# lawfuyang/HobbyRenderer

Hardware: AMD Instinct MI355X
Metric: Mrays/s at 1920×1080, 8 spp, 4 bounces; 1/2/4/8 GPU scaling (higher is better)
Workload: dtype f32; 1 GPU; config 2: Cornell-box-class procedural scene (38 triangles, 9 instances, closed room, emissive quad + default sun), 1920x1080, 8 spp (accumulation indices 0..7), 4 bounces; frames_in_flight=2, serial_kernels=False, mode=default

## Files before the change

### hobbyrenderer_amd/csrc/pt_device.h

```cpp
#pragma once

#include <hip/hip_runtime.h>
#include <stdint.h>

#include "../../include/hobbyrt_pt.h"
#include "../../include/hobbyrt/detmath.h"
#include "../../include/hobbyrt/srgb_table.h"

#define HRT_DEV __device__ __forceinline__

#if defined(HRPT_PHASE_PROFILE) && defined(HRPT_PHASE_TU)
extern __device__ unsigned long long g_phaseCounters[128];
#define HRT_PHASE(k)                                                                                                      \
    do {                                                                                                                  \
        const unsigned long long m_ = __ballot(true);                                                                     \
        if ((threadIdx.x & 63u) == (unsigned)(__ffsll((long long)m_) - 1)) {                                              \
            atomicAdd(&g_phaseCounters[2 * (k)], 1ull); atomicAdd(&g_phaseCounters[2 * (k) + 1], (unsigned long long)__popcll(m_)); \
        }                                                                                                                 \
    } while (0)
#else
#define HRT_PHASE(k) do { } while (0)
#endif
enum {
    PH_EXT_ITER = 0, PH_EXT_REFILL, PH_EXT_NODE, PH_EXT_LEAF, PH_EXT_TRI, PH_EXT_FINISH, PH_EXT_CANDIDATE,
    PH_ANY_ITER = 8, PH_ANY_REFILL, PH_ANY_NODE, PH_ANY_LEAF, PH_ANY_TRI, PH_ANY_FINISH,
    PH_SHADE_ITER = 16, PH_SHADE_HIT, PH_SHADE_ATTR, PH_SHADE_TEX, PH_SHADE_TRANS, PH_SHADE_NEE, PH_SHADE_LOBE_BEGIN, PH_SHADE_DIFFUSE, PH_SHADE_SPEC,
    PH_SHADE_SKY, PH_SHADE_WRITE, PH_SHADE_SORT,
    PH_SHADOW_ENTRY = 32, PH_SHADOW_SAMPLE, PH_SHADOW_QUERY, PH_SHADOW_CONTRIB, PH_SHADOW_RAYS_ITEM,
    PH_COUNT = 40
};

namespace hrt {

struct f2 { float x, y; };
struct f3 { float x, y, z; };
struct f4 { float x, y, z, w; };

HRT_DEV f3 mk3(float x, float y, float z) { f3 r; r.x = x; r.y = y; r.z = z; return r; }
HRT_DEV f3 mk3(const float* p) { return mk3(p[0], p[1], p[2]); }
HRT_DEV f3 operator+(f3 a, f3 b) { return mk3(a.x + b.x, a.y + b.y, a.z + b.z); }
HRT_DEV f3 operator-(f3 a, f3 b) { return mk3(a.x - b.x, a.y - b.y, a.z - b.z); }
HRT_DEV f3 operator*(f3 a, f3 b) { return mk3(a.x * b.x, a.y * b.y, a.z * b.z); }
HRT_DEV f3 operator*(f3 a, float s) { return mk3(a.x * s, a.y * s, a.z * s); }
HRT_DEV f3 operator/(f3 a, float s) { return mk3(a.x / s, a.y / s, a.z / s); }
HRT_DEV f3 operator-(f3 a) { return mk3(-a.x, -a.y, -a.z); }
HRT_DEV float dot(f3 a, f3 b) { return (a.x * b.x + a.y * b.y) + a.z * b.z; }
HRT_DEV f3 cross(f3 a, f3 b) { return mk3(a.y * b.z - a.z * b.y, a.z * b.x - a.x * b.z, a.x * b.y - a.y * b.x); }
HRT_DEV float length(f3 a) { return hrt_sqrt(dot(a, a)); }
HRT_DEV f3 normalize(f3 a) { float inv = 1.0f / hrt_sqrt(dot(a, a)); return a * inv; }
HRT_DEV float lerp(float a, float b, float t) { return a + t * (b - a); }
HRT_DEV float comp(f3 a, int k) { return k == 0 ? a.x : (k == 1 ? a.y : a.z); }
HRT_DEV float maxcomp(f3 a) { return hrt_max(a.x, hrt_max(a.y, a.z)); }
HRT_DEV f3 reflect(f3 i, f3 n) { float s = 2.0f * dot(i, n); return i - n * s; }
HRT_DEV f3 refract(f3 i, f3 n, float eta)
{
    float d = dot(n, i);
    float k = 1.0f - (eta * eta) * (1.0f - d * d);
    if (k < 0.0f) return mk3(0.0f, 0.0f, 0.0f);
    float s = eta * d + hrt_sqrt(k);
    return i * eta - n * s;
}
HRT_DEV f4 lerp4(f4 a, f4 b, float t)
{
    f4 r; float w = 1.0f - t;
    r.x = a.x * w + b.x * t; r.y = a.y * w + b.y * t; r.z = a.z * w + b.z * t; r.w = a.w * w + b.w * t;
    return r;
}

struct GpuNode {
    float lmin[3]; int32_t left;
    float lmax[3]; int32_t right;
    float rmin[3]; uint32_t pad0;
    float rmax[3]; uint32_t pad1;
};
struct GpuNode4 {
    float4 minx, maxx, miny, maxy, minz, maxz; int4 child; uint4 pad;
};
struct GpuNodeQ {
    float ox, oy, oz, sx;
    uint32_t lox, hix, loy, hiy;
    uint32_t loz, hiz; float sy, sz;
    int32_t child[4];
};
static_assert(sizeof(GpuNodeQ) == 64, "four 16-byte rows");
struct GpuTri {
    float p0[3]; uint32_t inst;
    float p1[3]; uint32_t prim;
    float p2[3]; uint32_t flags;
};
struct GpuTriAttr { float4 a, b, c, d, e; };
struct GpuTriTangent { float4 t0, t1, t2; };
struct GpuInstShade { float4 adj0, adj1, adj2; };
struct GpuInstance {
    float world[12];
    float inv[12];
    int32_t blasRoot; uint32_t flags, material; float boxEps;
    uint32_t mesh; float objMaxAbs, invNorm; uint32_t pad;
};
static_assert(sizeof(GpuInstance) == 128, "bvh_build.h HostInstance");
struct GpuTexture {
    const uint8_t* texels; uint32_t w, h, format, mipCount;
    uint32_t mipOffset[HRPT_TEXTURE_MAX_MIPS];
};

struct SceneView {
    const GpuNode* nodes; uint32_t nodeCount;
    const GpuNode4* nodes4; uint32_t node4Count;
    const GpuNodeQ* nodesQ;
    const GpuTri* tris; uint32_t triCount;
    int32_t rootLeaf;
    const GpuTriAttr* attrs;
    const GpuTriTangent* tangents;
    const GpuInstShade* instShade;
    const HrptMaterialConstants* materials;
    const HrptGPULight* lights; uint32_t lightCount;
    const GpuTexture* textures; uint32_t textureCount;
    const uint16_t* lutTransmittance;
    const uint16_t* lutScattering;
    const GpuInstance* instances; uint32_t instanceCount;
};

struct Ray { f3 o, d; float tmin, tmax; };
struct Hit { float t; uint32_t inst, prim; float u, v; uint32_t opaque; uint32_t tri; bool valid; };
struct HitKey { float t; uint32_t inst, prim; bool have; };

struct RayShear { int kx, ky, kz; float Sx, Sy, Sz; };

HRT_DEV RayShear make_shear(f3 d)
{
    RayShear s;
    int kz = 0;
    if (hrt_abs(d.y) > hrt_abs(comp(d, kz))) kz = 1;
    if (hrt_abs(d.z) > hrt_abs(comp(d, kz))) kz = 2;
    int kx = (kz + 1) % 3, ky = (kx + 1) % 3;
    if (comp(d, kz) < 0.0f) { int t = kx; kx = ky; ky = t; }
    s.kx = kx; s.ky = ky; s.kz = kz;
    float dz = comp(d, kz);
    s.Sx = comp(d, kx) / dz; s.Sy = comp(d, ky) / dz; s.Sz = 1.0f / dz;
    return s;
}
HRT_DEV bool key_less(float t, uint32_t inst, uint32_t prim, float t2, uint32_t inst2, uint32_t prim2)
{
    if (t < t2) return true;
    if (t > t2) return false;
    if (inst < inst2) return true;
    if (inst > inst2) return false;
    return prim < prim2;
}
HRT_DEV bool tri_test(f3 p0, f3 p1, f3 p2, const Ray& r, const RayShear& s, float& t, float& u, float& v)
{
    f3 A = p0 - r.o, B = p1 - r.o, C = p2 - r.o;
    float Akz = comp(A, s.kz), Bkz = comp(B, s.kz), Ckz = comp(C, s.kz);
    float Ax = comp(A, s.kx) - s.Sx * Akz, Ay = comp(A, s.ky) - s.Sy * Akz;
    float Bx = comp(B, s.kx) - s.Sx * Bkz, By = comp(B, s.ky) - s.Sy * Bkz;
    float Cx = comp(C, s.kx) - s.Sx * Ckz, Cy = comp(C, s.ky) - s.Sy * Ckz;
    float U = Cx * By - Cy * Bx;
    float V = Ax * Cy - Ay * Cx;
    float W = Bx * Ay - By * Ax;
    if ((U < 0.0f || V < 0.0f || W < 0.0f) && (U > 0.0f || V > 0.0f || W > 0.0f)) return false;
    float det = (U + V) + W;
    if (det == 0.0f) return false;
    float Az = s.Sz * Akz, Bz = s.Sz * Bkz, Cz = s.Sz * Ckz;
    float T = (U * Az + V * Bz) + W * Cz;
    float rcp = 1.0f / det;
    float tt = T * rcp;
    if (!(tt > r.tmin && tt < r.tmax)) return false;
    t = tt; u = V * rcp; v = W * rcp;
    return true;
}

struct GlobalBvh {
    static constexpr int kWidth = 2; static constexpr bool kTwoLevel = false;
    const GpuNode* nodes; const GpuTri* tris;
    HRT_DEV void node(int i, float4& a, float4& b, float4& c, float4& d) const
    {
        const float4* p = reinterpret_cast<const float4*>(nodes + i);
        a = p[0]; b = p[1]; c = p[2]; d = p[3];
    }
    HRT_DEV void tri(uint32_t i, float4& a, float4& b, float4& c) const
    {
        const float4* p = reinterpret_cast<const float4*>(tris + i);
        a = p[0]; b = p[1]; c = p[2];
    }
};

struct GlobalBvh4 {
    static constexpr int kWidth = 4; static constexpr bool kTwoLevel = false; static constexpr bool kLds = false;
    const GpuNode4* nodes; const GpuTri* tris;
    HRT_DEV void tri(uint32_t i, float4& a, float4& b, float4& c) const
    {
        const float4* p = reinterpret_cast<const float4*>(reinterpret_cast<const char*>(tris) + (size_t)(i * 48u));
        a = p[0]; b = p[1]; c = p[2];
    }
    HRT_DEV uint32_t rowoff(int i, uint32_t byteOffset) const { return (uint32_t)i * 128u + byteOffset; }
    HRT_DEV float4 load(uint32_t off) const { return *reinterpret_cast<const float4*>(reinterpret_cast<const char*>(nodes) + (size_t)off); }
};

struct GlobalBvhQ {
    static constexpr int kWidth = 4; static constexpr bool kTwoLevel = false; static constexpr bool kLds = false; static constexpr bool kQuantised = true;
    const GpuNodeQ* nodes; const GpuTri* tris;
    HRT_DEV void tri(uint32_t i, float4& a, float4& b, float4& c) const
    {
        const float4* p = reinterpret_cast<const float4*>(reinterpret_cast<const char*>(tris) + (size_t)(i * 48u));
        a = p[0]; b = p[1]; c = p[2];
    }
    HRT_DEV float4 row(int i, uint32_t r) const { return *reinterpret_cast<const float4*>(reinterpret_cast<const char*>(nodes) + (size_t)((uint32_t)i * 64u + r * 16u)); }
};
template <class BVH, class = void> struct IsQuantised { static constexpr bool value = false; };
template <class BVH> struct IsQuantised<BVH, decltype((void)BVH::kQuantised)> { static constexpr bool value = true; };

HRT_DEV f3 slab_origin_term(f3 o, f3 inv) { return mk3(-(o.x * inv.x), -(o.y * inv.y), -(o.z * inv.z)); }
HRT_DEV bool slab(float4 bmin, float4 bmax, f3 noi, f3 inv, float t0, float t1, float& tnear)
{
    float tx0 = __builtin_fmaf(bmin.x, inv.x, noi.x), tx1 = __builtin_fmaf(bmax.x, inv.x, noi.x);
    float ty0 = __builtin_fmaf(bmin.y, inv.y, noi.y), ty1 = __builtin_fmaf(bmax.y, inv.y, noi.y);
    float tz0 = __builtin_fmaf(bmin.z, inv.z, noi.z), tz1 = __builtin_fmaf(bmax.z, inv.z, noi.z);
    float lo = __builtin_fmaxf(__builtin_fmaxf(__builtin_fminf(tx0, tx1), __builtin_fminf(ty0, ty1)), __builtin_fmaxf(__builtin_fminf(tz0, tz1), t0));
    float hi = __builtin_fminf(__builtin_fminf(__builtin_fmaxf(tx0, tx1), __builtin_fmaxf(ty0, ty1)), __builtin_fminf(__builtin_fmaxf(tz0, tz1), t1));
    tnear = lo;
    return __builtin_fmaf(-__builtin_fabsf(lo), 2e-6f, lo) <= __builtin_fmaf(__builtin_fabsf(hi), 2e-6f, hi);
}

constexpr int32_t kTraversalDone = (int32_t)0x80000000;

HRT_DEV float slab1(float bminx, float bminy, float bminz, float bmaxx, float bmaxy, float bmaxz, f3 noi, f3 inv, float t0, float t1)
{
    float tx0 = __builtin_fmaf(bminx, inv.x, noi.x), tx1 = __builtin_fmaf(bmaxx, inv.x, noi.x);
    float ty0 = __builtin_fmaf(bminy, inv.y, noi.y), ty1 = __builtin_fmaf(bmaxy, inv.y, noi.y);
    float tz0 = __builtin_fmaf(bminz, inv.z, noi.z), tz1 = __builtin_fmaf(bmaxz, inv.z, noi.z);
    float lo = __builtin_fmaxf(__builtin_fmaxf(__builtin_fminf(tx0, tx1), __builtin_fminf(ty0, ty1)), __builtin_fmaxf(__builtin_fminf(tz0, tz1), t0));
    float hi = __builtin_fminf(__builtin_fminf(__builtin_fmaxf(tx0, tx1), __builtin_fmaxf(ty0, ty1)), __builtin_fminf(__builtin_fmaxf(tz0, tz1), t1));
    bool hit = __builtin_fmaf(-__builtin_fabsf(lo), 2e-6f, lo) <= __builtin_fmaf(__builtin_fabsf(hi), 2e-6f, hi);
    return hit ? lo : __builtin_inff();
}
HRT_DEV void cswap(float& ta, int32_t& ra, float& tb, int32_t& rb)
{
    bool sw = tb < ta;
    float t = sw ? tb : ta; tb = sw ? ta : tb; ta = t;
    int32_t r = sw ? rb : ra; rb = sw ? ra : rb; ra = r;
}

template <class BVH, class STACK>
HRT_DEV int32_t inner_step(const BVH& bvh, int32_t cur, f3 noi, f3 noiF, f3 inv, float tmin, float tlim, STACK& stack, int& sp)
{
    if constexpr (BVH::kWidth == 2) {
        float4 a, b, c, d; bvh.node(cur, a, b, c, d);
        int32_t li = __float_as_int(a.w), ri = __float_as_int(b.w);
        float tl, tr;
        bool hl = slab(a, b, noi, inv, tmin, tlim, tl);
        bool hr = slab(c, d, noi, inv, tmin, tlim, tr);
        if (hl && hr) { bool leftFirst = tl <= tr; stack.push(sp++, leftFirst ? ri : li); return leftFirst ? li : ri; }
        if (hl) return li;
        if (hr) return ri;
        return (sp == 0) ? kTraversalDone : stack.pop(--sp);
    } else if constexpr (IsQuantised<BVH>::value) {
        const float4 r0 = bvh.row(cur, 0u), r1 = bvh.row(cur, 1u), r2 = bvh.row(cur, 2u), chf = bvh.row(cur, 3u);
        const float ax = r0.w * inv.x, ay = r2.z * inv.y, az = r2.w * inv.z;
        const float bx = __builtin_fmaf(r0.x, inv.x, noi.x), by = __builtin_fmaf(r0.y, inv.y, noi.y), bz = __builtin_fmaf(r0.z, inv.z, noi.z);
        const bool negx = inv.x < 0.0f, negy = inv.y < 0.0f, negz = inv.z < 0.0f;
        const uint32_t wnx = __float_as_uint(negx ? r1.y : r1.x), wfx = __float_as_uint(negx ? r1.x : r1.y);
        const uint32_t wny = __float_as_uint(negy ? r1.w : r1.z), wfy = __float_as_uint(negy ? r1.z : r1.w);
        const uint32_t wnz = __float_as_uint(negz ? r2.y : r2.x), wfz = __float_as_uint(negz ? r2.x : r2.y);
        auto boxq = [&](uint32_t sh) {
            const float lo = __builtin_fmaxf(__builtin_fmaxf(__builtin_fmaxf(__builtin_fmaf((float)((wnx >> sh) & 255u), ax, bx), __builtin_fmaf((float)((wny >> sh) & 255u), ay, by)),
                                                             __builtin_fmaf((float)((wnz >> sh) & 255u), az, bz)), tmin);
            const float far3 = __builtin_fminf(__builtin_fminf(__builtin_fmaf((float)((wfx >> sh) & 255u), ax, bx), __builtin_fmaf((float)((wfy >> sh) & 255u), ay, by)),
                                               __builtin_fmaf((float)((wfz >> sh) & 255u), az, bz));
            const float hi = __builtin_fminf(far3, tlim) * (1.0f + 4e-6f);
            return lo <= hi ? lo : __builtin_inff();
        };
        float t0 = boxq(0u), t1 = boxq(8u), t2 = boxq(16u), t3 = boxq(24u);
        int32_t r0i = __float_as_int(chf.x), r1i = __float_as_int(chf.y), r2i = __float_as_int(chf.z), r3i = __float_as_int(chf.w);
        cswap(t0, r0i, t1, r1i); cswap(t2, r2i, t3, r3i); cswap(t0, r0i, t2, r2i); cswap(t1, r1i, t3, r3i); cswap(t1, r1i, t2, r2i);
        const float inf = __builtin_inff();
        if (t3 < inf) stack.push(sp++, r3i);
        if (t2 < inf) stack.push(sp++, r2i);
        if (t1 < inf) stack.push(sp++, r1i);
        if (t0 < inf) return r0i;
        return (sp == 0) ? kTraversalDone : stack.pop(--sp);
    } else {
        const uint32_t nx = inv.x < 0.0f ? 16u : 0u, ny = inv.y < 0.0f ? 48u : 32u, nz = inv.z < 0.0f ? 80u : 64u;
        const uint32_t onx = bvh.rowoff(cur, nx), ony = bvh.rowoff(cur, ny), onz = bvh.rowoff(cur, nz);
        const float4 anx = bvh.load(onx), any = bvh.load(ony), anz = bvh.load(onz);
        const float4 afx = bvh.load(onx ^ 16u), afy = bvh.load(ony ^ 16u), afz = bvh.load(onz ^ 16u);
        const float4 chf = bvh.load(bvh.rowoff(cur, 96u));
        auto box = [&](float bnx, float bny, float bnz, float bfx, float bfy, float bfz) {
            const float lo = __builtin_fmaxf(__builtin_fmaxf(__builtin_fmaxf(__builtin_fmaf(bnx, inv.x, noi.x), __builtin_fmaf(bny, inv.y, noi.y)), __builtin_fmaf(bnz, inv.z, noi.z)), tmin);
            const float far3 = __builtin_fminf(__builtin_fminf(__builtin_fmaf(bfx, inv.x, noiF.x), __builtin_fmaf(bfy, inv.y, noiF.y)), __builtin_fmaf(bfz, inv.z, noiF.z));
            const float hi = __builtin_fminf(far3, tlim) * (1.0f + 4e-6f);
            return lo <= hi ? lo : __builtin_inff();
        };
        float t0 = box(anx.x, any.x, anz.x, afx.x, afy.x, afz.x);
        float t1 = box(anx.y, any.y, anz.y, afx.y, afy.y, afz.y);
        float t2 = box(anx.z, any.z, anz.z, afx.z, afy.z, afz.z);
        float t3 = box(anx.w, any.w, anz.w, afx.w, afy.w, afz.w);
        int32_t r0 = __float_as_int(chf.x), r1 = __float_as_int(chf.y), r2 = __float_as_int(chf.z), r3 = __float_as_int(chf.w);
        cswap(t0, r0, t1, r1); cswap(t2, r2, t3, r3); cswap(t0, r0, t2, r2); cswap(t1, r1, t3, r3); cswap(t1, r1, t2, r2);
        const float inf = __builtin_inff();
        if (t3 < inf) stack.push(sp++, r3);
        if (t2 < inf) stack.push(sp++, r2);
        if (t1 < inf) stack.push(sp++, r1);
        if (t0 < inf) return r0;
        return (sp == 0) ? kTraversalDone : stack.pop(--sp);
    }
}

template <class BVH, class STACK>
HRT_DEV int32_t inner_step(const BVH& bvh, int32_t cur, f3 noi, f3 inv, float tmin, float tlim, STACK& stack, int& sp)
{
    return inner_step(bvh, cur, noi, noi, inv, tmin, tlim, stack, sp);
}

HRT_DEV f3 traversal_rcp(f3 d)
{
    auto one = [](float x) { return __builtin_fminf(__builtin_fmaxf(__builtin_amdgcn_rcpf(x), -1e20f), 1e20f); };
    return mk3(one(d.x), one(d.y), one(d.z));
}

template <class BVH, class STACK>
HRT_DEV Hit closest_any(const BVH& bvh, int32_t rootLeaf, uint32_t nodeCount, const Ray& r, HitKey lower, STACK& stack, uint32_t nodeLoopMin = 0)
{
    Hit best; best.valid = false; best.t = r.tmax; best.inst = 0; best.prim = 0; best.u = 0; best.v = 0; best.opaque = 0; best.tri = 0;
    if (!(r.d.x == r.d.x && r.d.y == r.d.y && r.d.z == r.d.z)) return best;
    RayShear sh = make_shear(r.d);
    f3 inv = traversal_rcp(r.d), noi = slab_origin_term(r.o, inv);
    int sp = 0;
    int32_t cur;
    if (nodeCount == 0) { if (rootLeaf == 0) return best; cur = rootLeaf; }
    else cur = 0;
    float tlim = r.tmax;
    for (;;) {
        while (cur >= 0) {
            cur = inner_step(bvh, cur, noi, inv, r.tmin, tlim, stack, sp);
            if ((uint32_t)__popcll(__ballot(cur >= 0)) < nodeLoopMin) break;
        }
        if (cur == kTraversalDone) break;
        if (cur < 0) {
            uint32_t enc = (uint32_t)(~cur);
            uint32_t first = enc >> 2, count = (enc & 3u) + 1u;
            for (uint32_t i = 0; i < count; ++i) {
                float4 a, b, c; bvh.tri(first + i, a, b, c);
                float t, u, v;
                if (tri_test(mk3(a.x, a.y, a.z), mk3(b.x, b.y, b.z), mk3(c.x, c.y, c.z), r, sh, t, u, v)) {
                    uint32_t inst = __float_as_uint(a.w), prim = __float_as_uint(b.w);
                    bool ok = !lower.have || key_less(lower.t, lower.inst, lower.prim, t, inst, prim);
                    const bool take = ok && (!best.valid || key_less(t, inst, prim, best.t, best.inst, best.prim));
                    best.t = take ? t : best.t; best.u = take ? u : best.u; best.v = take ? v : best.v;
                    best.inst = take ? inst : best.inst; best.prim = take ? prim : best.prim; best.tri = take ? first + i : best.tri;
                    best.opaque = take ? (__float_as_uint(c.w) & 1u) : best.opaque;
                    best.valid = best.valid || take;
                    tlim = take ? t : tlim;
                }
            }
            if (sp == 0) break;
            cur = stack.pop(--sp);
        }
    }
    return best;
}

template <class BVH, class STACK>
HRT_DEV bool any_opaque(const BVH& bvh, int32_t rootLeaf, uint32_t nodeCount, const Ray& r, STACK& stack, bool& sawNonOpaque, uint32_t nodeLoopMin = 0)
{
    sawNonOpaque = false;
    if (!(r.d.x == r.d.x && r.d.y == r.d.y && r.d.z == r.d.z)) return false;
    RayShear sh = make_shear(r.d);
    f3 inv = traversal_rcp(r.d), noi = slab_origin_term(r.o, inv);
    int sp = 0; int32_t cur;
    if (nodeCount == 0) { if (rootLeaf == 0) return false; cur = rootLeaf; }
    else cur = 0;
    for (;;) {
        while (cur >= 0) {
            cur = inner_step(bvh, cur, noi, inv, r.tmin, r.tmax, stack, sp);
            if ((uint32_t)__popcll(__ballot(cur >= 0)) < nodeLoopMin) break;
        }
        if (cur == kTraversalDone) break;
        if (cur < 0) {
            uint32_t enc = (uint32_t)(~cur);
            uint32_t first = enc >> 2, count = (enc & 3u) + 1u;
            for (uint32_t i = 0; i < count; ++i) {
                float4 a, b, c; bvh.tri(first + i, a, b, c);
                float t, u, v;
                if (tri_test(mk3(a.x, a.y, a.z), mk3(b.x, b.y, b.z), mk3(c.x, c.y, c.z), r, sh, t, u, v)) {
                    if (__float_as_uint(c.w) & 1u) return true;
                    sawNonOpaque = true;
                }
            }
            if (sp == 0) break;
            cur = stack.pop(--sp);
        }
    }
    return false;
}

constexpr int32_t kExitBlas = 0x7FFFFFFE;
struct GlobalBvhTl : GlobalBvh4 {
    static constexpr bool kTwoLevel = true;
    const GpuInstance* instances;
};
struct TlCull { f3 inv, noi, noiF; int32_t inst; };
HRT_DEV void tl_world(TlCull& c, const Ray& r)
{
    c.inv = traversal_rcp(r.d); c.noi = slab_origin_term(r.o, c.inv); c.noiF = c.noi; c.inst = -1;
}
HRT_DEV void tl_enter(TlCull& c, const GpuInstance& I, int32_t inst, const Ray& r)
{
    const float4* w = reinterpret_cast<const float4*>(I.world);
    const float4 w2 = w[2];
    const float4* q = reinterpret_cast<const float4*>(I.inv);
    const float4 q0 = q[0], q1 = q[1]; const float q22 = I.inv[8];
    const f3 rel = mk3(r.o.x - w2.y, r.o.y - w2.z, r.o.z - w2.w);
    const f3 oo = mk3(__builtin_fmaf(rel.z, q1.z, __builtin_fmaf(rel.y, q0.w, rel.x * q0.x)),
                      __builtin_fmaf(rel.z, q1.w, __builtin_fmaf(rel.y, q1.x, rel.x * q0.y)),
                      __builtin_fmaf(rel.z, q22, __builtin_fmaf(rel.y, q1.y, rel.x * q0.z)));
    const f3 od = mk3(__builtin_fmaf(r.d.z, q1.z, __builtin_fmaf(r.d.y, q0.w, r.d.x * q0.x)),
                      __builtin_fmaf(r.d.z, q1.w, __builtin_fmaf(r.d.y, q1.x, r.d.x * q0.y)),
                      __builtin_fmaf(r.d.z, q22, __builtin_fmaf(r.d.y, q1.y, r.d.x * q0.z)));
    auto max3abs = [](f3 v) { return __builtin_fmaxf(__builtin_fmaxf(__builtin_fabsf(v.x), __builtin_fabsf(v.y)), __builtin_fabsf(v.z)); };
    const float oMax = __builtin_fmaxf(max3abs(r.o), __builtin_fmaxf(__builtin_fmaxf(__builtin_fabsf(w2.y), __builtin_fabsf(w2.z)), __builtin_fabsf(w2.w)));
    const float dRatio = max3abs(r.d) * I.invNorm / __builtin_fmaxf(max3abs(od), 1e-30f);
    const float eps = I.boxEps + 4.0f * 2.4e-7f * (I.invNorm * (oMax + max3abs(rel)) + dRatio * (I.objMaxAbs + max3abs(oo)));
    c.inv = traversal_rcp(od);
    const f3 n = slab_origin_term(oo, c.inv);
    const f3 e = mk3(eps * __builtin_fabsf(c.inv.x), eps * __builtin_fabsf(c.inv.y), eps * __builtin_fabsf(c.inv.z));
    c.noi = mk3(n.x - e.x, n.y - e.y, n.z - e.z); c.noiF = mk3(n.x + e.x, n.y + e.y, n.z + e.z);
    c.inst = inst;
}
HRT_DEV void tl_world_triangle(const GpuInstance& I, float4 a, float4 b, float4 c, f3& p0, f3& p1, f3& p2)
{
    const float4* w = reinterpret_cast<const float4*>(I.world);
    const float4 w0 = w[0], w1 = w[1], w2 = w[2];
    auto xf = [&](float x, float y, float z) {
        return mk3(((x * w0.x + y * w0.w) + z * w1.z) + w2.y,
                   ((x * w0.y + y * w1.x) + z * w1.w) + w2.z,
                   ((x * w0.z + y * w1.y) + z * w2.x) + w2.w);
    };
    p0 = xf(a.x, a.y, a.z); p1 = xf(b.x, b.y, b.z); p2 = xf(c.x, c.y, c.z);
}
template <class STACK>
HRT_DEV int32_t tl_switch(const GlobalBvhTl& bvh, int32_t cur, TlCull& c, const Ray& r, STACK& stack, int& sp)
{
    if (cur == kExitBlas) { tl_world(c, r); return sp == 0 ? kTraversalDone : stack.pop(--sp); }
    const int32_t inst = (int32_t)(((uint32_t)~cur) >> 2);
    const GpuInstance& I = bvh.instances[inst];
    const int32_t root = I.blasRoot;
    if (root == kTraversalDone) return sp == 0 ? kTraversalDone : stack.pop(--sp);
    stack.push(sp++, kExitBlas);
    tl_enter(c, I, inst, r);
    return root;
}

template <class STACK>
HRT_DEV bool any_hit_two_level(const GlobalBvhTl& bvh, int32_t rootLeaf, uint32_t nodeCount, const Ray& r, STACK& stack, bool& sawNonOpaque, uint32_t nodeLoopMin = 0)
{
    sawNonOpaque = false;
    if (!(r.d.x == r.d.x && r.d.y == r.d.y && r.d.z == r.d.z)) return false;
    RayShear sh = make_shear(r.d);
    TlCull c; tl_world(c, r);
    int sp = 0; int32_t cur;
    if (nodeCount == 0) { if (rootLeaf == 0) return false; cur = rootLeaf; }
    else cur = 0;
    for (;;) {
        while (cur >= 0 && cur != kExitBlas) {
            cur = inner_step(bvh, cur, c.noi, c.noiF, c.inv, r.tmin, r.tmax, stack, sp);
            if ((uint32_t)__popcll(__ballot(cur >= 0 && cur != kExitBlas)) < nodeLoopMin) break;
        }
        if (cur == kTraversalDone) break;
        if (cur == kExitBlas || (cur < 0 && c.inst < 0)) { cur = tl_switch(bvh, cur, c, r, stack, sp); continue; }
        if (cur < 0) {
            const GpuInstance& I = bvh.instances[c.inst];
            uint32_t enc = (uint32_t)(~cur);
            uint32_t first = enc >> 2, count = (enc & 3u) + 1u;
            for (uint32_t i = 0; i < count; ++i) {
                float4 ta, tb, tc; bvh.tri(first + i, ta, tb, tc);
                f3 p0, p1, p2; tl_world_triangle(I, ta, tb, tc, p0, p1, p2);
                float t, u, v;
                if (tri_test(p0, p1, p2, r, sh, t, u, v)) { if (I.flags & 1u) return true; sawNonOpaque = true; }
            }
            cur = stack.pop(--sp);
        }
    }
    return false;
}
template <class STACK>
HRT_DEV Hit closest_two_level(const GlobalBvhTl& bvh, int32_t rootLeaf, uint32_t nodeCount, const Ray& r, HitKey lower, STACK& stack)
{
    Hit best; best.valid = false; best.t = r.tmax; best.inst = 0; best.prim = 0; best.u = 0; best.v = 0; best.opaque = 0; best.tri = 0;
    if (!(r.d.x == r.d.x && r.d.y == r.d.y && r.d.z == r.d.z)) return best;
    RayShear sh = make_shear(r.d);
    TlCull c; tl_world(c, r);
    int sp = 0; int32_t cur;
    if (nodeCount == 0) { if (rootLeaf == 0) return best; cur = rootLeaf; }
    else cur = 0;
    float tlim = r.tmax;
    for (;;) {
        while (cur >= 0 && cur != kExitBlas) cur = inner_step(bvh, cur, c.noi, c.noiF, c.inv, r.tmin, tlim, stack, sp);
        if (cur == kTraversalDone) break;
        if (cur == kExitBlas || (cur < 0 && c.inst < 0)) { cur = tl_switch(bvh, cur, c, r, stack, sp); continue; }
        const GpuInstance& I = bvh.instances[c.inst];
        const uint32_t enc = (uint32_t)(~cur), first = enc >> 2, count = (enc & 3u) + 1u, inst = (uint32_t)c.inst;
        for (uint32_t i = 0; i < count; ++i) {
            float4 ta, tb, tc; bvh.tri(first + i, ta, tb, tc);
            f3 p0, p1, p2; tl_world_triangle(I, ta, tb, tc, p0, p1, p2);
            float t, u, v;
            const bool hitTri = tri_test(p0, p1, p2, r, sh, t, u, v);
            const uint32_t prim = __float_as_uint(tb.w);
            const bool ok = !lower.have || key_less(lower.t, lower.inst, lower.prim, t, inst, prim);
            const bool take = hitTri && ok && (!best.valid || key_less(t, inst, prim, best.t, best.inst, best.prim));
            best.t = take ? t : best.t; best.u = take ? u : best.u; best.v = take ? v : best.v;
            best.inst = take ? inst : best.inst; best.prim = take ? prim : best.prim; best.tri = take ? first + i : best.tri;
            best.opaque = take ? (I.flags & 1u) : best.opaque;
            best.valid = best.valid || take;
            tlim = take ? t : tlim;
        }
        cur = stack.pop(--sp);
    }
    return best;
}

struct TriVerts { f3 n0, n1, n2; f2 uv0, uv1, uv2; uint32_t material, inst; };
HRT_DEV TriVerts unpack_tri_attr(const float4* p)
{
    float4 a = p[0], b = p[1], c = p[2], d = p[3], e = p[4];
    TriVerts t;
    t.n0 = mk3(a.x, a.y, a.z); t.n1 = mk3(a.w, b.x, b.y); t.n2 = mk3(b.z, b.w, c.x);
    t.uv0.x = c.y; t.uv0.y = c.z; t.uv1.x = c.w; t.uv1.y = d.x; t.uv2.x = d.y; t.uv2.y = d.z;
    t.material = __float_as_uint(d.w); t.inst = __float_as_uint(e.x);
    return t;
}
HRT_DEV TriVerts load_tri_attr(const SceneView& s, uint32_t tri) { return unpack_tri_attr(reinterpret_cast<const float4*>(s.attrs + tri)); }
HRT_DEV TriVerts load_hit_attr(const SceneView& s, const Hit& hit)
{
    TriVerts tv = load_tri_attr(s, hit.tri);
    if (s.instances) { tv.inst = hit.inst; tv.material = s.instances[hit.inst].material; }
    return tv;
}
HRT_DEV f2 interpolated_uv(const TriVerts& tv, float bx, float by)
// ... 601 lines not shown
```

### hobbyrenderer_amd/csrc/pt_path.h

```cpp
#pragma once

#include "pt_device.h"

namespace hrt {

struct PathState {
    Ray ray;
    uint32_t rng;
    f3 throughput, radiance;
    bool inVolume; float interiorIOR; f3 sigmaA, sigmaS;
};

struct SurfaceCarry {
    f3 N, V, worldPos, baseColor, F0; float Fr, roughness, metallic, ior;
    uint32_t rngBeforeLights;
    uint32_t material;
};

HRT_DEV void init_path(PathState& ps, const HrptPathTracerConstants& cb, uint32_t px, uint32_t py)
{
    float u = (((float)px + 0.5f) + cb.m_Jitter[0]) * cb.m_View.m_ViewportSizeInv[0];
    float v = (((float)py + 0.5f) + cb.m_Jitter[1]) * cb.m_View.m_ViewportSizeInv[1];
    float cx = u * 2.0f + -1.0f, cy = v * -2.0f + 1.0f;
    const float* M = cb.m_View.m_MatClipToWorldNoOffset;
// ... 101 lines not shown
                    f3 p0, p1, p2; tl_world_triangle(s.instances[h.inst], tp[0], tp[1], tp[2], p0, p1, p2);
                    const float w0 = (1.0f - h.u) - h.v;
                    const f3 hitPos = (p0 * w0 + p1 * h.u) + p2 * h.v;
                    const float dist = length(hitPos - ray.o);
                    const float triangleArea = length(cross(p1 - p0, p2 - p0)) * 0.5f;
                    f2 uvRange;
                    uvRange.x = hrt_max(tv.uv0.x, hrt_max(tv.uv1.x, tv.uv2.x)) - hrt_min(tv.uv0.x, hrt_min(tv.uv1.x, tv.uv2.x));
                    uvRange.y = hrt_max(tv.uv0.y, hrt_max(tv.uv1.y, tv.uv2.y)) - hrt_min(tv.uv0.y, hrt_min(tv.uv1.y, tv.uv2.y));
                    const float gradientScale = triangleArea / hrt_max(dist, 0.1f);
                    f2 grad; grad.x = uvRange.x * gradientScale; grad.y = uvRange.y * gradientScale;
                    alpha *= sample_texture_grad(t, mat.m_AlbedoSamplerIndex, uv, grad, grad).w;
                }
            }
        }
        return alpha >= mat.m_AlphaCutoff;
    }
    if (mat.m_AlphaMode != HRPT_ALPHA_MODE_BLEND) return true;
    float alpha = candidate_alpha(s, mat, uv);
    float opacity = hrt_saturate(alpha * (1.0f - mat.m_TransmissionFactor));
    st.transmission *= (1.0f - opacity);
    if (mat.m_TransmissionFactor > 0.0f && mat.m_IsThinSurface == 0) {
        float w0 = (1.0f - h.u) - h.v;
        f3 ln = (tv.n0 * w0 + tv.n1 * h.u) + tv.n2 * h.v;
        f3 wn = normalize(transform_normal(ln, s.instShade[tv.inst]));
        bool front = dot(wn, ray.d) < 0.0f;
        if (front) { st.inVolume = true; st.inVolumeStartT = h.t; st.sigmaT = mk3(mat.m_SigmaA) + mk3(mat.m_SigmaS); }
        else if (st.inVolume) {
            float seg = hrt_max(0.0f, h.t - st.inVolumeStartT);
            f3 tr = mk3(hrt_exp(-st.sigmaT.x * seg), hrt_exp(-st.sigmaT.y * seg), hrt_exp(-st.sigmaT.z * seg));
            st.transmission *= dot(tr, mk3(0.2126f, 0.7152f, 0.0722f));
            st.inVolume = false;
        }
    }
    return st.transmission <= 1e-3f;
}
template <class STACK>
HRT_DEV float shadow_retrace_two_level(const SceneView& s, const GlobalBvhTl& bvh, const Ray& ray, STACK& stack)
{
    ShadowState st; st.transmission = 1.0f; st.inVolume = false; st.inVolumeStartT = 0.0f; st.sigmaT = mk3(0.0f, 0.0f, 0.0f);
    HitKey lower; lower.have = false; lower.t = 0.0f; lower.inst = 0; lower.prim = 0;
    for (;;) {
        Hit h = closest_two_level(bvh, s.rootLeaf, s.nodeCount, ray, lower, stack);
        if (!h.valid) break;
        if (h.opaque) return 0.0f;
        if (shadow_candidate_two_level(s, ray, h, st)) return 0.0f;
        lower.have = true; lower.t = h.t; lower.inst = h.inst; lower.prim = h.prim;
    }
    return shadow_finish(ray, st);
}
template <int K, class STACK, class CAND3>
HRT_DEV float shadow_query_two_level_buffered(const SceneView& s, const GlobalBvhTl& bvh, const Ray& ray, STACK& stack, CAND3& cand, uint32_t nodeLoopMin = 0)
{
    if (!(ray.d.x == ray.d.x && ray.d.y == ray.d.y && ray.d.z == ray.d.z)) return 1.0f;
    RayShear sh = make_shear(ray.d);
    TlCull c; tl_world(c, ray);
    int sp = 0, count = 0; bool overflow = false;
    int32_t cur;
    if (s.nodeCount == 0) { if (s.rootLeaf == 0) return 1.0f; cur = s.rootLeaf; } else cur = 0;
    auto prim_of = [&](uint32_t tri) { return reinterpret_cast<const uint32_t*>(bvh.tris + tri)[7]; };
    for (;;) {
        while (cur >= 0 && cur != kExitBlas) {
            cur = inner_step(bvh, cur, c.noi, c.noiF, c.inv, ray.tmin, ray.tmax, stack, sp);
            if ((uint32_t)__popcll(__ballot(cur >= 0 && cur != kExitBlas)) < nodeLoopMin) break;
        }
        if (cur == kTraversalDone) break;
        if (cur == kExitBlas || (cur < 0 && c.inst < 0)) { cur = tl_switch(bvh, cur, c, ray, stack, sp); continue; }
        if (cur >= 0) continue;
        const GpuInstance& I = bvh.instances[c.inst];
        const uint32_t enc = (uint32_t)(~cur), first = enc >> 2, n = (enc & 3u) + 1u, inst = (uint32_t)c.inst;
        for (uint32_t i = 0; i < n; ++i) {
            float4 ta, tb, tc; bvh.tri(first + i, ta, tb, tc);
            f3 p0, p1, p2; tl_world_triangle(I, ta, tb, tc, p0, p1, p2);
            float t, u, v;
            if (!tri_test(p0, p1, p2, ray, sh, t, u, v)) continue;
            if (I.flags & 1u) return 0.0f;
            const uint32_t prim = __float_as_uint(tb.w);
            int pos = count;
            if (count == K) {
                float lt; uint32_t ltri, linst; cand.key(K - 1, lt, ltri, linst);
                overflow = true;
                if (!key_less(t, inst, prim, lt, linst, prim_of(ltri))) continue;
                pos = K - 1;
            } else ++count;
            while (pos > 0) {
                float pt; uint32_t ptri, pinst; cand.key(pos - 1, pt, ptri, pinst);
                const bool less = t != pt ? t < pt : key_less(t, inst, prim, pt, pinst, prim_of(ptri));
                if (!less) break;
                cand.move(pos, pos - 1);
                --pos;
            }
            cand.set(pos, t, first + i, inst);
        }
        cur = stack.pop(--sp);
    }
    if (count == 0) return 1.0f;
    ShadowState st; st.transmission = 1.0f; st.inVolume = false; st.inVolumeStartT = 0.0f; st.sigmaT = mk3(0.0f, 0.0f, 0.0f);
    Hit h; h.valid = true; h.opaque = 0; h.t = 0.0f; h.u = 0.0f; h.v = 0.0f; h.tri = 0; h.inst = 0; h.prim = 0;
    for (int k = 0; k < count; ++k) {
        float kt; cand.key(k, kt, h.tri, h.inst);
        float4 ta, tb, tc; bvh.tri(h.tri, ta, tb, tc);
        f3 p0, p1, p2; tl_world_triangle(bvh.instances[h.inst], ta, tb, tc, p0, p1, p2);
        tri_test(p0, p1, p2, ray, sh, h.t, h.u, h.v);
        h.prim = __float_as_uint(tb.w);
        if (shadow_candidate_two_level(s, ray, h, st)) return 0.0f;
    }
    if (overflow) {
        HitKey lower; lower.have = true; lower.t = h.t; lower.inst = h.inst; lower.prim = h.prim;
        for (;;) {
            Hit n = closest_two_level(bvh, s.rootLeaf, s.nodeCount, ray, lower, stack);
            if (!n.valid) break;
            if (n.opaque) return 0.0f;
            if (shadow_candidate_two_level(s, ray, n, st)) return 0.0f;
            lower.t = n.t; lower.inst = n.inst; lower.prim = n.prim;
        }
    }
    return shadow_finish(ray, st);
}
template <class STACK>
HRT_DEV float shadow_query_two_level(const SceneView& s, const GlobalBvhTl& bvh, const Ray& ray, STACK& stack, uint32_t nodeLoopMin = 0)
{
    bool sawNonOpaque;
    if (any_hit_two_level(bvh, s.rootLeaf, s.nodeCount, ray, stack, sawNonOpaque, nodeLoopMin)) return 0.0f;
    return sawNonOpaque ? shadow_retrace_two_level(s, bvh, ray, stack) : 1.0f;
}

template <bool ALL_OPAQUE = false, class BVH, class STACK>
HRT_DEV float shadow_query(const SceneView& s, const BVH& bvh, f3 worldPos, f3 L, float maxDist, STACK& stack, uint32_t nodeLoopMin = 0)
{
    Ray ray = shadow_ray(worldPos, L, maxDist);
    if constexpr (BVH::kTwoLevel) {
        if constexpr (ALL_OPAQUE) { bool none; return any_hit_two_level(bvh, s.rootLeaf, s.nodeCount, ray, stack, none, nodeLoopMin) ? 0.0f : 1.0f; }
        else return shadow_query_two_level(s, bvh, ray, stack, nodeLoopMin);
    }
    bool sawNonOpaque;
    if (any_opaque(bvh, s.rootLeaf, s.nodeCount, ray, stack, sawNonOpaque, nodeLoopMin)) return 0.0f;
    if (ALL_OPAQUE || !sawNonOpaque) return 1.0f;
    ShadowState st; st.transmission = 1.0f; st.inVolume = false; st.inVolumeStartT = 0.0f; st.sigmaT = mk3(0.0f, 0.0f, 0.0f);
    HitKey lower; lower.have = false; lower.t = 0.0f; lower.inst = 0; lower.prim = 0;
    for (;;) {
        Hit h = closest_any(bvh, s.rootLeaf, s.nodeCount, ray, lower, stack);
        if (!h.valid) break;
        if (shadow_candidate(s, ray, h.t, h.tri, h.u, h.v, st)) return 0.0f;
        lower.have = true; lower.t = h.t; lower.inst = h.inst; lower.prim = h.prim;
    }
    return shadow_finish(ray, st);
}

template <int K, class BVH, class CAND>
HRT_DEV void candidate_insert(const BVH& bvh, CAND& cand, int& count, bool& overflow, float t, uint32_t tri, uint32_t inst, uint32_t prim)
{
    int pos = count;
    if (count == K) {
        float lt; uint32_t ltri; cand.key(K - 1, lt, ltri);
        float4 la, lb, lc; bvh.tri(ltri, la, lb, lc);
        overflow = true;
        if (!key_less(t, inst, prim, lt, __float_as_uint(la.w), __float_as_uint(lb.w))) return;
        pos = K - 1;
    } else ++count;
    while (pos > 0) {
        float pt; uint32_t ptri; cand.key(pos - 1, pt, ptri);
        bool less;
        if (t != pt) less = t < pt;
        else { float4 pa, pb, pc; bvh.tri(ptri, pa, pb, pc); less = key_less(t, inst, prim, pt, __float_as_uint(pa.w), __float_as_uint(pb.w)); }
        if (!less) break;
        cand.move(pos, pos - 1);
        --pos;
    }
    cand.set(pos, t, tri);
}
template <class BVH, class STACK, class CAND>
HRT_DEV float shadow_resolve_candidates(const SceneView& s, const BVH& bvh, const Ray& ray, const RayShear& sh, int count, bool overflow, const CAND& cand, STACK& stack)
{
    if (count == 0) return 1.0f;
    ShadowState st; st.transmission = 1.0f; st.inVolume = false; st.inVolumeStartT = 0.0f; st.sigmaT = mk3(0.0f, 0.0f, 0.0f);
    float lastT = 0.0f; uint32_t lastTri = 0;
    for (int k = 0; k < count; ++k) {
        float t; uint32_t tri; cand.key(k, t, tri);
        float4 a, b, c; bvh.tri(tri, a, b, c);
        float t2, u, v;
        tri_test(mk3(a.x, a.y, a.z), mk3(b.x, b.y, b.z), mk3(c.x, c.y, c.z), ray, sh, t2, u, v);
        if (shadow_candidate(s, ray, t, tri, u, v, st)) return 0.0f;
        lastT = t; lastTri = tri;
    }
    if (overflow) {
        float4 la, lb, lc; bvh.tri(lastTri, la, lb, lc);
        HitKey lower; lower.have = true; lower.t = lastT; lower.inst = __float_as_uint(la.w); lower.prim = __float_as_uint(lb.w);
        for (;;) {
            Hit h = closest_any(bvh, s.rootLeaf, s.nodeCount, ray, lower, stack);
            if (!h.valid) break;
            if (h.opaque) return 0.0f;
            if (shadow_candidate(s, ray, h.t, h.tri, h.u, h.v, st)) return 0.0f;
            lower.t = h.t; lower.inst = h.inst; lower.prim = h.prim;
        }
    }
    return shadow_finish(ray, st);
}
template <int K, class BVH, class STACK, class CAND>
HRT_DEV float shadow_query_buffered(const SceneView& s, const BVH& bvh, f3 worldPos, f3 L, float maxDist, STACK& stack, CAND& cand, uint32_t nodeLoopMin = 0)
{
    Ray ray = shadow_ray(worldPos, L, maxDist);
    if (!(ray.d.x == ray.d.x && ray.d.y == ray.d.y && ray.d.z == ray.d.z)) return 1.0f;
    RayShear sh = make_shear(ray.d);
    f3 inv = traversal_rcp(ray.d), noi = slab_origin_term(ray.o, inv);
    int sp = 0, count = 0; bool overflow = false;
    int32_t cur;
    if (s.nodeCount == 0) { if (s.rootLeaf == 0) return 1.0f; cur = s.rootLeaf; } else cur = 0;
    for (;;) {
        while (cur >= 0) {
            cur = inner_step(bvh, cur, noi, inv, ray.tmin, ray.tmax, stack, sp);
            if ((uint32_t)__popcll(__ballot(cur >= 0)) < nodeLoopMin) break;
        }
        if (cur == kTraversalDone) break;
        if (cur >= 0) continue;
        uint32_t enc = (uint32_t)(~cur);
        uint32_t first = enc >> 2, n = (enc & 3u) + 1u;
        for (uint32_t i = 0; i < n; ++i) {
            float4 a, b, c; bvh.tri(first + i, a, b, c);
            float t, u, v;
            if (!tri_test(mk3(a.x, a.y, a.z), mk3(b.x, b.y, b.z), mk3(c.x, c.y, c.z), ray, sh, t, u, v)) continue;
            if (__float_as_uint(c.w) & 1u) return 0.0f;
            candidate_insert<K>(bvh, cand, count, overflow, t, first + i, __float_as_uint(a.w), __float_as_uint(b.w));
        }
        if (sp == 0) break;
        cur = stack.pop(--sp);
    }
    return shadow_resolve_candidates(s, bvh, ray, sh, count, overflow, cand, stack);
}

template <bool DIRONLY>
HRT_DEV bool nee_draw(const HrptGPULight& l, f3 N, f3 worldPos, f3 sunDirection, uint32_t& rng, float& ux, float& uy)
{
    if (DIRONLY || l.m_Type == HRPT_LIGHT_DIRECTIONAL) {
        if (dot(N, sunDirection) <= 0.0f) return false;
    } else if (!DIRONLY && (l.m_Type == HRPT_LIGHT_POINT || l.m_Type == HRPT_LIGHT_SPOT)) {
        if (l.m_Intensity <= 0.0f) return false;
        f3 toLight = mk3(l.m_Position) - worldPos;
        float distSq = dot(toLight, toLight);
        if (l.m_Range > 0.0f && distSq > l.m_Range * l.m_Range) return false;
        if (l.m_Type == HRPT_LIGHT_SPOT) {
            float dist = hrt_sqrt(distSq);
            f3 Lc = toLight / dist;
            if (dot(N, Lc) <= 0.0f) return false;
            f3 lightDir = normalize(mk3(l.m_Direction));
            float cosTheta = dot(-Lc, lightDir);
            if (cosTheta < hrt_cos(l.m_SpotOuterConeAngle)) return false;
        }
    } else return false;
    ux = hrt_rng_next(&rng); uy = hrt_rng_next(&rng);
    return true;
}

template <bool DIRONLY>
HRT_DEV bool nee_direction(const HrptGPULight& l, f3 N, f3 worldPos, f3 sunDirection, float cosSun, float ux, float uy, f3& L, float& maxDist)
{
    if (DIRONLY || l.m_Type == HRPT_LIGHT_DIRECTIONAL) {
        L = sample_cone(sunDirection, cosSun, ux, uy);
        maxDist = 1e10f;
    } else {
        float cosT = 1.0f - 2.0f * ux;
        float sinT = hrt_sqrt(hrt_max(0.0f, 1.0f - cosT * cosT));
        float phi = 2.0f * HRT_PI * uy;
        float sp, cp; hrt_sincos(phi, &sp, &cp);
        f3 sphereDir = mk3(sinT * cp, cosT, sinT * sp);
        f3 samplePos = mk3(l.m_Position) + sphereDir * l.m_Radius;
        f3 toSample = samplePos - worldPos;
        float sampleDist = length(toSample);
        L = toSample / sampleDist;
        maxDist = sampleDist;
    }
    return !(dot(N, L) <= 0.0f);
}

template <bool DIRONLY>
HRT_DEV void nee_contribution(const SceneView& s, const HrptGPULight& l, Lighting in, f3 worldPos, f3 sunDirection, float sunIntensity, f3 L,
                              f3& diffuse, f3& specular)
{
    f3 radiance;
    if (DIRONLY || l.m_Type == HRPT_LIGHT_DIRECTIONAL) {
        radiance = atm::sun_radiance(s, atm::atmosphere_pos(worldPos), sunDirection, sunIntensity);
    } else {
        f3 toLight = mk3(l.m_Position) - worldPos;
        float distSq = dot(toLight, toLight);
        float dist = hrt_sqrt(distSq);
        float att = distance_attenuation(l, distSq, dist);
        f3 col = mk3(l.m_Color);
        if (l.m_Type == HRPT_LIGHT_SPOT) {
            f3 Lc = toLight / dist;
            f3 lightDir = normalize(mk3(l.m_Direction));
            float cosTheta = dot(-Lc, lightDir);
            float cosOuter = hrt_cos(l.m_SpotOuterConeAngle), cosInner = hrt_cos(l.m_SpotInnerConeAngle);
            float spotAtt = hrt_saturate((cosTheta - cosOuter) / (cosInner - cosOuter));
            radiance = ((col * l.m_Intensity) * spotAtt) * att;
        } else radiance = (col * l.m_Intensity) * att;
    }
    in.L = L;
    prepare_byproducts(in);
    evaluate_direct_unshadowed(in, radiance, diffuse, specular);
}

HRT_DEV Lighting nee_lighting(f3 N, f3 V, f3 baseColor, float roughness, float metallic, float ior)
{
    Lighting in;
    in.N = N; in.V = V; in.L = mk3(0.0f, 0.0f, 0.0f); in.baseColor = baseColor; in.roughness = roughness; in.metallic = metallic; in.ior = ior;
    return in;
}

HRT_DEV HrptGPULight load_light(const SceneView& s, uint32_t i)
{
    if (i < s.lightCount) return s.lights[i];
    HrptGPULight l = HrptGPULight(); l.m_Type = 0;
    return l;
}

enum SurfaceOutcome { SURFACE_TRANSMITTED = 0, SURFACE_SCATTER = 1 };

template <bool TEX, bool TRANS, bool DIRONLY, class TABLES, class EMIT>
HRT_DEV SurfaceOutcome shade_surface_a(const SceneView& s, const TABLES& tables, const HrptPathTracerConstants& cb, PathState& ps, const Hit& hit,
                                       SurfaceCarry& carry, EMIT&& emit)
{
    TriVerts tv = tables.hit_attr(hit);
    GpuInstShade is = tables.inst_shade(tv.inst);
    const HrptMaterialConstants& mat = tables.material(tv.material);
    uint32_t texFlags = TEX ? mat.m_TextureFlags : 0u;

    if (TRANS && ps.inVolume) {
        f3 tr = mk3(hrt_exp(-(ps.sigmaA.x + ps.sigmaS.x) * hit.t), hrt_exp(-(ps.sigmaA.y + ps.sigmaS.y) * hit.t),
                    hrt_exp(-(ps.sigmaA.z + ps.sigmaS.z) * hit.t));
        ps.throughput = ps.throughput * tr;
    }
    SurfaceAttr attr = full_hit_attributes(s, hit, ps.ray, tv, is, (texFlags & HRPT_TEXFLAG_NORMAL) != 0);
    Pbr pbr = pbr_attributes(s, attr, mat, texFlags);

    f3 Ng = normalize(attr.worldNormal);
    f3 N = pbr.normal;
    f3 V = -ps.ray.d;
    bool isFrontFace = dot(Ng, ps.ray.d) < 0.0f;
    if (dot(N, V) < 0.0f) N = -N;

    f3 sunDir = mk3(cb.m_SunDirection[0], cb.m_SunDirection[1], cb.m_SunDirection[2]);

    Lighting in;
    in.N = N; in.V = V; in.L = mk3(0.0f, 0.0f, 0.0f); in.baseColor = pbr.baseColor;
    in.roughness = pbr.roughness; in.metallic = pbr.metallic; in.ior = mat.m_IOR;
    prepare_byproducts(in);

    HRT_PHASE(PH_SHADE_ATTR);
    if (TRANS && (mat.m_TransmissionFactor > 0.0f || mat.m_AlphaMode == HRPT_ALPHA_MODE_BLEND)) {
        HRT_PHASE(PH_SHADE_TRANS);
        float effectiveAlpha = (mat.m_AlphaMode == HRPT_ALPHA_MODE_BLEND) ? pbr.alpha : 1.0f;
        float transmissionFactor = hrt_max(mat.m_TransmissionFactor, 1.0f - effectiveAlpha);
        float materialIOR = hrt_max(mat.m_IOR, 1.0001f);
        float outsideIOR = ps.inVolume ? ps.interiorIOR : 1.0f;
        float etaSurface = isFrontFace ? (outsideIOR / materialIOR) : (materialIOR / outsideIOR);
        float etaFresnel = etaSurface;
        float etaRefract = (mat.m_IsThinSurface != 0) ? 1.0f : etaFresnel;
        float cosT_geo;
        float F = fresnel_dielectric(etaFresnel, hrt_max(dot(N, V), 0.0f), cosT_geo);
        float probT = hrt_saturate((1.0f - F) * transmissionFactor);
        if (hrt_rng_next(&ps.rng) < probT) {
            f3 refractedDir, bsdfWeight;
            if (pbr.roughness <= 0.08f) {
                refractedDir = refract(ps.ray.d, N, etaRefract);
                if (dot(refractedDir, refractedDir) < 1e-8f) refractedDir = reflect(ps.ray.d, N);
                bsdfWeight = pbr.baseColor;
            } else {
                float ux = hrt_rng_next(&ps.rng), uy = hrt_rng_next(&ps.rng);
                f3 H = sample_ggx_vndf(ux, uy, N, V, pbr.roughness);
                float VdotH = hrt_saturate(dot(V, H));
                float cosT_mf; float F_mf = fresnel_dielectric(etaFresnel, VdotH, cosT_mf);
                float cosT_dir; fresnel_dielectric(etaRefract, VdotH, cosT_dir);
                refractedDir = H * (etaRefract * VdotH - cosT_dir) - V * etaRefract;
                if (dot(refractedDir, refractedDir) < 1e-8f) refractedDir = reflect(ps.ray.d, H);
                refractedDir = normalize(refractedDir);
                float alpha = pbr.roughness * pbr.roughness, alpha2 = alpha * alpha;
// ... 89 lines not shown
```

### hobbyrenderer_amd/csrc/pt_wavefront.hip

```cpp
#define HRPT_PHASE_TU 1
#include "pt_wavefront.h"

#include <mutex>
#include <type_traits>
#include <unordered_map>
#include <vector>

#include "bvh_build.h"
#include "pt_gbuffer.h"
#include "pt_motion.h"
#include "pt_path.h"

#ifdef HRPT_PHASE_PROFILE
__device__ unsigned long long g_phaseCounters[128];
#endif
#ifdef HRPT_SKY_DEBUG
__device__ float g_skyDebug[2048 * 16];
#endif

namespace hrt {

namespace {

constexpr uint32_t kMaxSppPerBatch = 64;

struct WfBuffers {
    float4 *rayO[2], *rayD[2], *thr[2], *med0[2], *med1[2];
    uint32_t* pathCnt[2];
    float4* hit;
    uint32_t* hitInst;
    float4 *sh0, *sh1, *sh2, *sh3, *sh4, *shL;
    uint32_t* shadowCnt;
    float4 *sqO, *sqD; uint32_t* sqId; uint32_t* sqCnt; uint32_t* shVis;
    uint2* sqCand;
    float4* radiance;
};

struct WfArgs {
    SceneView scene;
    WfBuffers b;
    uint32_t segSize;
    uint32_t numSegments;
    uint32_t numSamples;
    uint32_t pixelsPadded;
    uint32_t tilesX, tilesY;
    TileRect rect;
    uint32_t imageWidth;
    uint32_t spp;
    uint32_t maxLights;
    uint32_t hasMedium;
    uint32_t hasStochasticAlpha;
    uint32_t allOpaque;
    uint32_t refillMin;
    uint32_t streamSegments;
    uint32_t slimShadow;
    uint32_t shadowParity;
    uint32_t nodeLoopMin;
    uint32_t sortShade;
    uint32_t shadeInstances, shadeMaterials;
    const struct PrimaryArgs* primaryArgs;
    uint32_t primary;
    int32_t* spill[2];
    DeviceCounters* counters;
};

enum : uint32_t { kVisNoRay = 0, kVisBlocked = 1, kVisClear = 2, kVisCandidates = 3 };

struct JitterTable { float2 j[kMaxSppPerBatch]; };
struct PrimaryArgs { float clipToWorld[16]; float cam[3]; float invW, invH; uint32_t accumIndex; float2 j[kMaxSppPerBatch]; };

HRT_DEV void tile_position(const WfArgs& a, uint32_t tile, uint32_t& tcol, uint32_t& trow)
{
    if (a.rect.stripeCount > 1u) { tcol = tile / a.tilesY; trow = tile - tcol * a.tilesY; }
    else { trow = tile / a.tilesX; tcol = tile - trow * a.tilesX; }
}

HRT_DEV bool primary_ray(const WfArgs& a, const PrimaryArgs& pr, uint32_t smp, f3& o, f3& d, uint32_t& rng)
{
    const uint32_t k = smp / a.pixelsPadded, p = smp - k * a.pixelsPadded;
    const uint32_t tile = p >> 6, within = p & 63u;
    uint32_t tcol, trow; tile_position(a, tile, tcol, trow);
    const uint32_t px = a.rect.column_x(tcol) + (within & 7u), py = a.rect.y0 + trow * 8u + (within >> 3);
    if (!(px < a.rect.x1 && py < a.rect.y1)) return false;
    const float u = (((float)px + 0.5f) + pr.j[k].x) * pr.invW;
    const float v = (((float)py + 0.5f) + pr.j[k].y) * pr.invH;
    const float cx = u * 2.0f + -1.0f, cy = v * -2.0f + 1.0f;
    const float* M = pr.clipToWorld;
    const float ex = ((cx * M[0] + cy * M[4]) + 0.9f * M[8]) + 1.0f * M[12];
    const float ey = ((cx * M[1] + cy * M[5]) + 0.9f * M[9]) + 1.0f * M[13];
    const float ez = ((cx * M[2] + cy * M[6]) + 0.9f * M[10]) + 1.0f * M[14];
    const float ew = ((cx * M[3] + cy * M[7]) + 0.9f * M[11]) + 1.0f * M[15];
    const f3 end = mk3(ex / ew, ey / ew, ez / ew);
    o = mk3(pr.cam[0], pr.cam[1], pr.cam[2]);
    d = normalize(end - o);
    rng = hrt_rng_seed(px, py, pr.accumIndex + k);
    return true;
}
HRT_DEV uint32_t path_count(const WfArgs& a, uint32_t in, uint32_t seg)
{
    (void)in;
    const uint32_t base = seg * a.segSize, left = a.numSamples - base, size = a.segSize; return left < size ? left : size;
}

template <int DEPTH, int LDSMAX>
struct LdsStack {
    static constexpr int kLdsStackMax = LDSMAX;
    static constexpr int kLds = DEPTH > kLdsStackMax ? kLdsStackMax : DEPTH;
    static constexpr int kRows = kLds;
    int32_t* base; int32_t* spill; uint32_t spillStride;
    HRT_DEV void push(int sp, int32_t v)
    {
        if (DEPTH <= kLdsStackMax || sp < kLds) base[(sp & (kLds - 1)) * kBlock] = v;
        else spill[(size_t)(sp - kLds) * spillStride] = v;
    }
    HRT_DEV int32_t pop(int sp)
    {
        if (DEPTH <= kLdsStackMax || sp < kLds) return base[(sp & (kLds - 1)) * kBlock];
        return spill[(size_t)(sp - kLds) * spillStride];
    }
};
struct LdsCandidates {
    int32_t* base;
    HRT_DEV void key(int k, float& t, uint32_t& tri) const { t = __int_as_float(base[(k * 2 + 0) * kBlock]); tri = (uint32_t)base[(k * 2 + 1) * kBlock]; }
    HRT_DEV void set(int k, float t, uint32_t tri) { base[(k * 2 + 0) * kBlock] = __float_as_int(t); base[(k * 2 + 1) * kBlock] = (int32_t)tri; }
    HRT_DEV void move(int dst, int src) { base[(dst * 2 + 0) * kBlock] = base[(src * 2 + 0) * kBlock]; base[(dst * 2 + 1) * kBlock] = base[(src * 2 + 1) * kBlock]; }
};
struct LdsCandidates3 {
    int32_t* base;
    HRT_DEV void key(int k, float& t, uint32_t& tri, uint32_t& inst) const { t = __int_as_float(base[(k * 3 + 0) * kBlock]); tri = (uint32_t)base[(k * 3 + 1) * kBlock]; inst = (uint32_t)base[(k * 3 + 2) * kBlock]; }
    HRT_DEV void set(int k, float t, uint32_t tri, uint32_t inst) { base[(k * 3 + 0) * kBlock] = __float_as_int(t); base[(k * 3 + 1) * kBlock] = (int32_t)tri; base[(k * 3 + 2) * kBlock] = (int32_t)inst; }
    HRT_DEV void move(int dst, int src) { for (int w = 0; w < 3; ++w) base[(dst * 3 + w) * kBlock] = base[(src * 3 + w) * kBlock]; }
};
struct GlobalCandidates {
    const uint2* base;
    HRT_DEV void key(int k, float& t, uint32_t& tri) const { uint2 v = base[k]; t = __uint_as_float(v.x); tri = v.y; }
};
template <int W>
struct LdsBvh {
    static constexpr int kWidth = W == 5 ? 4 : W; static constexpr bool kTwoLevel = false; static constexpr bool kLds = true;
    const float4* nodes; const float4* tris;
    HRT_DEV void node(int i, float4& a, float4& b, float4& c, float4& d) const { const float4* p = nodes + 4 * i; a = p[0]; b = p[1]; c = p[2]; d = p[3]; }
    HRT_DEV void tri(uint32_t i, float4& a, float4& b, float4& c) const { const float4* p = tris + 3 * i; a = p[0]; b = p[1]; c = p[2]; }
    typedef __attribute__((address_space(3))) const char* LdsPtr;
    HRT_DEV uint32_t rowoff(int i, uint32_t byteOffset) const { return (uint32_t)(uintptr_t)(LdsPtr) reinterpret_cast<const char*>(nodes) + (uint32_t)i * kLdsNode4Stride + byteOffset; }
    HRT_DEV float4 load(uint32_t off) const { return *reinterpret_cast<const float4*>((const char*)(LdsPtr)(uintptr_t)off); }
};
template <int W> struct GlobalBvhOf;
template <> struct GlobalBvhOf<2> { using type = GlobalBvh; static HRT_DEV GlobalBvh make(const SceneView& s) { GlobalBvh g; g.nodes = s.nodes; g.tris = s.tris; return g; } };
constexpr int kTwoLevelTree = 44;
template <> struct GlobalBvhOf<kTwoLevelTree> { using type = GlobalBvhTl; static HRT_DEV GlobalBvhTl make(const SceneView& s) { GlobalBvhTl g; g.nodes = s.nodes4; g.tris = s.tris; g.instances = s.instances; return g; } };
template <> struct GlobalBvhOf<4> { using type = GlobalBvh4; static HRT_DEV GlobalBvh4 make(const SceneView& s) { GlobalBvh4 g; g.nodes = s.nodes4; g.tris = s.tris; return g; } };
constexpr int kQuantisedTree = 5;
template <> struct GlobalBvhOf<kQuantisedTree> { using type = GlobalBvhQ; static HRT_DEV GlobalBvhQ make(const SceneView& s) { GlobalBvhQ g; g.nodes = s.nodesQ; g.tris = s.tris; return g; } };

template <bool LDS_BVH, int DEPTH, int W, int LDSMAX>
HRT_DEV void setup_lds(char* smem, const SceneView& s, LdsStack<DEPTH, LDSMAX>& stack, LdsBvh<W>& lbvh, size_t extraBytes = 0)
{
    stack.base = reinterpret_cast<int32_t*>(smem) + threadIdx.x;
    stack.spill = nullptr; stack.spillStride = 0;
    if (LDS_BVH) {
        float4* dst = reinterpret_cast<float4*>(smem + (size_t)LdsStack<DEPTH, LDSMAX>::kRows * kBlock * 4 + extraBytes);
        const float4* srcN = W == 2 ? reinterpret_cast<const float4*>(s.nodes) : reinterpret_cast<const float4*>(s.nodes4);
        const float4* srcT = reinterpret_cast<const float4*>(s.tris);
        uint32_t nN = W == 2 ? s.nodeCount * 4 : s.node4Count * 8, nT = s.triCount * 3;
        uint32_t nNdst = nN;
        if (W == 2 || kLdsNode4Stride == 128u) { for (uint32_t i = threadIdx.x; i < nN; i += kBlock) dst[i] = srcN[i]; }
        else { nNdst = s.node4Count * (kLdsNode4Stride / 16u); for (uint32_t i = threadIdx.x; i < nN; i += kBlock) dst[(i >> 3) * (kLdsNode4Stride / 16u) + (i & 7u)] = srcN[i]; }
        for (uint32_t i = threadIdx.x; i < nT; i += kBlock) dst[nNdst + i] = srcT[i];
        lbvh.nodes = dst; lbvh.tris = dst + nNdst;
        __syncthreads();
    }
}

HRT_DEV uint32_t lane_id() { return threadIdx.x & 63u; }
HRT_DEV uint32_t uniform(uint32_t v) { return (uint32_t)__builtin_amdgcn_readfirstlane((int)v); }
HRT_DEV uint32_t prefix_rank(unsigned long long mask) { return __builtin_amdgcn_mbcnt_hi((uint32_t)(mask >> 32), __builtin_amdgcn_mbcnt_lo((uint32_t)mask, 0u)); }

HRT_DEV unsigned long long wave_sum_u32(unsigned int v)
{
    unsigned long long x = v;
#pragma unroll
    for (int off = 32; off > 0; off >>= 1) x += __shfl_xor(x, off, 64);
    return x;
}
HRT_DEV void block_count_add(unsigned long long* counterField0, size_t fieldOffsetWords, unsigned int perLane)
{
    __shared__ unsigned long long partial[kBlock / 64];
    unsigned long long w = wave_sum_u32(perLane);
    if (lane_id() == 0) partial[threadIdx.x >> 6] = w;
    __syncthreads();
    if (threadIdx.x == 0) {
        unsigned long long t = 0;
        for (uint32_t i = 0; i < kBlock / 64; ++i) t += partial[i];
        if (t) atomicAdd(counterField0 + (size_t)(blockIdx.x % kCounterShards) * (sizeof(DeviceCounters) / 8) + fieldOffsetWords, t);
    }
}
template <int N>
HRT_DEV void block_count_add_uniform(DeviceCounters* counters, const int (&fields)[N], const unsigned int (&perWave)[N])
{
    __shared__ unsigned int partialU[N][kBlock / 64];
    if (lane_id() == 0)
        for (int k = 0; k < N; ++k) partialU[k][threadIdx.x >> 6] = perWave[k];
    __syncthreads();
    if (threadIdx.x < (uint32_t)N) {
        unsigned long long t = 0;
        for (uint32_t i = 0; i < kBlock / 64; ++i) t += partialU[threadIdx.x][i];
        if (t) atomicAdd(reinterpret_cast<unsigned long long*>(counters + blockIdx.x % kCounterShards) + fields[threadIdx.x], t);
    }
}

__global__ void wf_store_primary(PrimaryArgs pr, PrimaryArgs* dst)
{
    if (threadIdx.x < 16) dst->clipToWorld[threadIdx.x] = pr.clipToWorld[threadIdx.x];
    if (threadIdx.x < 3) dst->cam[threadIdx.x] = pr.cam[threadIdx.x];
    if (threadIdx.x == 0) { dst->invW = pr.invW; dst->invH = pr.invH; dst->accumIndex = pr.accumIndex; }
    if (threadIdx.x < kMaxSppPerBatch) dst->j[threadIdx.x] = pr.j[threadIdx.x];
}

__global__ __launch_bounds__(kBlock) void wf_raygen(WfArgs a, HrptPathTracerConstants cb, JitterTable jt)
{
    const uint32_t wavesPerBlock = kBlock / 64, lane = lane_id();
    const uint32_t gw = uniform(blockIdx.x * wavesPerBlock + (threadIdx.x >> 6)), totalWaves = gridDim.x * wavesPerBlock;
    unsigned int nPaths = 0;
    for (uint32_t seg = gw; seg < a.numSegments; seg += totalWaves) {
        uint32_t segBase = seg * a.segSize, outCount = 0;
        for (uint32_t base = 0; base < a.segSize; base += 64) {
            uint32_t smp = segBase + base + lane;
            const bool mine = base + lane < a.segSize && smp < a.numSamples;
            bool active = mine;
            uint32_t k = 0, px = 0, py = 0;
            if (active) {
                k = smp / a.pixelsPadded;
                uint32_t p = smp - k * a.pixelsPadded;
                uint32_t tile = p >> 6, within = p & 63u;
                uint32_t tcol, trow; tile_position(a, tile, tcol, trow);
                px = a.rect.column_x(tcol) + (within & 7u);
                py = a.rect.y0 + trow * 8u + (within >> 3);
                active = px < a.rect.x1 && py < a.rect.y1;
            }
            if (mine) a.b.radiance[smp] = make_float4(0.0f, 0.0f, 0.0f, 0.0f);
            unsigned long long m = __ballot(active);
            if (active) {
                PathState ps;
                {
                    float u = (((float)px + 0.5f) + jt.j[k].x) * cb.m_View.m_ViewportSizeInv[0];
                    float v = (((float)py + 0.5f) + jt.j[k].y) * cb.m_View.m_ViewportSizeInv[1];
                    float cx = u * 2.0f + -1.0f, cy = v * -2.0f + 1.0f;
                    const float* M = cb.m_View.m_MatClipToWorldNoOffset;
                    float ex = ((cx * M[0] + cy * M[4]) + 0.9f * M[8]) + 1.0f * M[12];
                    float ey = ((cx * M[1] + cy * M[5]) + 0.9f * M[9]) + 1.0f * M[13];
                    float ez = ((cx * M[2] + cy * M[6]) + 0.9f * M[10]) + 1.0f * M[14];
                    float ew = ((cx * M[3] + cy * M[7]) + 0.9f * M[11]) + 1.0f * M[15];
                    f3 end = mk3(ex / ew, ey / ew, ez / ew);
                    ps.ray.o = mk3(cb.m_CameraPos[0], cb.m_CameraPos[1], cb.m_CameraPos[2]);
                    ps.ray.d = normalize(end - ps.ray.o);
                    ps.rng = hrt_rng_seed(px, py, cb.m_AccumulationIndex + k);
                }
                uint32_t o = segBase + outCount + prefix_rank(m);
                a.b.rayO[0][o] = make_float4(ps.ray.o.x, ps.ray.o.y, ps.ray.o.z, 0.0f);
                a.b.rayD[0][o] = make_float4(ps.ray.d.x, ps.ray.d.y, ps.ray.d.z, __uint_as_float(ps.rng));
                a.b.thr[0][o] = make_float4(1.0f, 1.0f, 1.0f, __uint_as_float(smp));
                if (a.hasMedium) {
                    a.b.med0[0][o] = make_float4(0.0f, 0.0f, 0.0f, 1.0f);
                    a.b.med1[0][o] = make_float4(0.0f, 0.0f, 0.0f, 0.0f);
                }
                ++nPaths;
            }
            outCount += (uint32_t)__popcll(m);
        }
        if (lane == 0) a.b.pathCnt[0][seg] = outCount;
    }
    block_count_add(&a.counters->closestRays, 2, nPaths);
}

constexpr int kWavesExtendLds = 6, kWavesExtendGlobal = 6, kWavesExtendTwoLevel = 5, kWavesShade = 4;
#ifndef HRPT_WAVES_EXTEND_LDS_OPAQUE
#define HRPT_WAVES_EXTEND_LDS_OPAQUE 6
#endif
constexpr int kWavesExtendLdsOpaque = HRPT_WAVES_EXTEND_LDS_OPAQUE;
static_assert(sizeof(GpuTriAttr) == kTriAttrBytes && sizeof(GpuInstShade) == kInstShadeBytes && sizeof(HrptMaterialConstants) == kMaterialBytes, "pt_wavefront_plan.h shade_table_bytes");
constexpr uint32_t kNoPathRecord = 0xFFFFFFFEu;

template <bool LDS_BVH, int DEPTH, int W, bool ANYHIT, int TL = 0, bool PRIMARY = false, bool OPQ = false>
__global__ __launch_bounds__(kBlock) __attribute__((amdgpu_waves_per_eu(TL ? kWavesExtendTwoLevel : (LDS_BVH ? (OPQ ? kWavesExtendLdsOpaque : kWavesExtendLds) : kWavesExtendGlobal)))) void wf_extend(WfArgs a, uint32_t parity)
{
    static_assert(!OPQ || (!ANYHIT && !TL), "OPQ: closest hits over the flat structure");
    static_assert(!TL || (!LDS_BVH && !ANYHIT && W == 4), "two-level traversal: global 4-wide tree, closest hit");
    static_assert(!PRIMARY || !ANYHIT, "primary rays are closest-hit rays");
    static_assert(W != kQuantisedTree || (!LDS_BVH && !TL), "quantised nodes: flat tree in global memory");
    extern __shared__ __attribute__((aligned(128))) char smem[];
    LdsStack<DEPTH, kExtendLdsStack> stack; LdsBvh<W> lbvh;
    constexpr size_t candBytes = ANYHIT ? (size_t)kShadowCandidates * 2 * kBlock * 4 : 0;
    setup_lds<LDS_BVH, DEPTH, W>(smem, a.scene, stack, lbvh, candBytes);
    LdsCandidates cand; cand.base = reinterpret_cast<int32_t*>(smem + (size_t)LdsStack<DEPTH, kExtendLdsStack>::kRows * kBlock * 4) + threadIdx.x;
    if (DEPTH > kExtendLdsStack) { stack.spill = a.spill[ANYHIT ? 1 : 0] + blockIdx.x * kBlock + threadIdx.x; stack.spillStride = gridDim.x * kBlock; }
    typename GlobalBvhOf<(TL ? kTwoLevelTree : W)>::type gbvh = GlobalBvhOf<(TL ? kTwoLevelTree : W)>::make(a.scene);
    const SceneView& s = a.scene;

    const uint32_t wavesPerBlock = kBlock / 64;
    const uint32_t gw = uniform(blockIdx.x * wavesPerBlock + (threadIdx.x >> 6)), totalWaves = gridDim.x * wavesPerBlock;
    const float4* __restrict__ rayO = ANYHIT ? a.b.sqO : a.b.rayO[parity];
    float4* __restrict__ rayD = ANYHIT ? a.b.sqD : a.b.rayD[parity];
    const uint32_t* __restrict__ segCount = ANYHIT ? a.b.sqCnt : a.b.pathCnt[parity];
    const uint32_t slotsPerSample = ANYHIT ? a.maxLights : 1u;
    unsigned int nRays = 0;
    const bool emptyScene = s.nodeCount == 0 && s.rootLeaf == 0;

    {
        uint32_t seg = gw, cnt = 0, segBase = 0, next = 0;
        bool haveSeg = false;
        auto open_segment = [&]() {
            haveSeg = false; cnt = 0; next = 0;
            for (; seg < a.numSegments; seg += totalWaves) {
                cnt = uniform(PRIMARY ? path_count(a, 0u, seg) : segCount[seg]);
                if (cnt) { segBase = (seg * a.segSize) * slotsPerSample; haveSeg = true; break; }
            }
        };
        open_segment();
        bool active = false;
        Ray r; r.o = mk3(0.0f, 0.0f, 0.0f); r.d = mk3(0.0f, 0.0f, 1.0f); r.tmin = 0.0f; r.tmax = 1e10f;
        RayShear sh = make_shear(r.d); f3 inv = mk3(0.0f, 0.0f, 0.0f), noi = mk3(0.0f, 0.0f, 0.0f);
        TlCull tl; tl.inv = inv; tl.noi = noi; tl.noiF = noi; tl.inst = -1;
        HitKey lower; lower.have = false; lower.t = 0.0f; lower.inst = 0; lower.prim = 0;
        Hit best; best.valid = false; best.t = 0.0f; best.inst = 0; best.prim = 0; best.u = 0.0f; best.v = 0.0f; best.opaque = 0; best.tri = 0;
        int32_t cur = kTraversalDone; int sp = 0; uint32_t slot = 0, rng = 0, rng0 = 0; float tlim = 0.0f;
        bool blocked = false, candOverflow = false; int candCount = 0;
        for (;;) {
            if (haveSeg && next >= cnt && (a.streamSegments || __ballot(active) == 0ull)) { seg += totalWaves; open_segment(); }
            unsigned long long mIdle = __ballot(!active);
            uint32_t nIdle = (uint32_t)__popcll(mIdle);
            if (active) HRT_PHASE(ANYHIT ? PH_ANY_ITER : PH_EXT_ITER);
            if (haveSeg && (nIdle >= a.refillMin || nIdle == 64u)) {
                const uint32_t idx = next + prefix_rank(mIdle);
                bool take = !active && idx < cnt;
                if constexpr (PRIMARY) {
                    if (take) {
                        slot = segBase + idx; take = primary_ray(a, *a.primaryArgs, slot, r.o, r.d, rng); r.tmin = 0.0f; r.tmax = 1e10f; rng0 = rng;
                        if (take) rayD[slot] = make_float4(r.d.x, r.d.y, r.d.z, __uint_as_float(rng));
                        else a.b.hit[slot] = make_float4(0.0f, 0.0f, 0.0f, __uint_as_float(kNoPathRecord));
                    }
                }
                if (take) {
                    HRT_PHASE(ANYHIT ? PH_ANY_REFILL : PH_EXT_REFILL);
                    if constexpr (!PRIMARY) {
                        slot = segBase + idx;
                        float4 o = rayO[slot], d = rayD[slot];
                        r.o = mk3(o.x, o.y, o.z); r.d = mk3(d.x, d.y, d.z); r.tmin = o.w; r.tmax = ANYHIT ? d.w : 1e10f;
                        rng = __float_as_uint(d.w); rng0 = rng;
                    }
                    blocked = false; candOverflow = false; candCount = 0;
                    lower.have = false;
                    best.valid = false; tlim = r.tmax; sp = 0;
                    bool finite = (r.d.x == r.d.x && r.d.y == r.d.y && r.d.z == r.d.z);
                    sh = make_shear(r.d);
                    if constexpr (TL) tl_world(tl, r); else { inv = traversal_rcp(r.d); noi = slab_origin_term(r.o, inv); }
                    cur = (emptyScene || !finite) ? kTraversalDone : (s.nodeCount == 0 ? s.rootLeaf : 0);
                    active = true; ++nRays;
                }
                next += nIdle;
            }
            if (__ballot(active) == 0ull) { if (haveSeg) continue; break; }
            if (active) {
                if constexpr (TL) {
                    while (cur >= 0 && cur != kExitBlas) {
                        cur = inner_step(gbvh, cur, tl.noi, tl.noiF, tl.inv, r.tmin, tlim, stack, sp);
                        if ((uint32_t)__popcll(__ballot(cur >= 0 && cur != kExitBlas)) < a.nodeLoopMin) break;
                    }
                    if (cur == kExitBlas || (cur < 0 && cur != kTraversalDone && tl.inst < 0)) cur = tl_switch(gbvh, cur, tl, r, stack, sp);
                    else if (cur < 0 && cur != kTraversalDone) {
                        const GpuInstance& I = s.instances[tl.inst];
                        const uint32_t enc = (uint32_t)(~cur), first = enc >> 2, count = (enc & 3u) + 1u;
                        const uint32_t inst = (uint32_t)tl.inst, iflags = I.flags & 7u;
                        for (uint32_t i = 0; i < count; ++i) {
                            float4 ta, tb, tc; gbvh.tri(first + i, ta, tb, tc);
                            f3 p0, p1, p2; tl_world_triangle(I, ta, tb, tc, p0, p1, p2);
                            float t, u, v;
                            const bool hitTri = tri_test(p0, p1, p2, r, sh, t, u, v);
                            const uint32_t prim = __float_as_uint(tb.w);
                            const bool ok = TL != 2 || !lower.have || key_less(lower.t, lower.inst, lower.prim, t, inst, prim);
                            const bool take = hitTri && ok && (!best.valid || key_less(t, inst, prim, best.t, best.inst, best.prim));
                            best.t = take ? t : best.t; best.u = take ? u : best.u; best.v = take ? v : best.v;
                            best.inst = take ? inst : best.inst; best.prim = take ? prim : best.prim; best.tri = take ? first + i : best.tri;
                            best.opaque = take ? iflags : best.opaque;
                            best.valid = best.valid || take;
                            tlim = take ? t : tlim;
                        }
                        cur = stack.pop(--sp);
                    }
                } else {
                while (cur >= 0) {
                    HRT_PHASE(ANYHIT ? PH_ANY_NODE : PH_EXT_NODE);
                    if (LDS_BVH) cur = inner_step(lbvh, cur, noi, inv, r.tmin, tlim, stack, sp);
                    else cur = inner_step(gbvh, cur, noi, inv, r.tmin, tlim, stack, sp);
                    if ((uint32_t)__popcll(__ballot(cur >= 0)) < a.nodeLoopMin) break;
                }
                }
                if (!TL && cur < 0 && cur != kTraversalDone) {
                    uint32_t enc = (uint32_t)(~cur);
                    uint32_t first = enc >> 2, count = (enc & 3u) + 1u;
                    HRT_PHASE(ANYHIT ? PH_ANY_LEAF : PH_EXT_LEAF);
                    for (uint32_t i = 0; i < count; ++i) {
                        HRT_PHASE(ANYHIT ? PH_ANY_TRI : PH_EXT_TRI);
                        float4 ta, tb, tc;
                        if (LDS_BVH) lbvh.tri(first + i, ta, tb, tc); else gbvh.tri(first + i, ta, tb, tc);
                        float t, u, v;
                        if (tri_test(mk3(ta.x, ta.y, ta.z), mk3(tb.x, tb.y, tb.z), mk3(tc.x, tc.y, tc.z), r, sh, t, u, v)) {
                            if (ANYHIT) {
                                if (__float_as_uint(tc.w) & 1u) { blocked = true; break; }
                                if (LDS_BVH) candidate_insert<kShadowCandidates>(lbvh, cand, candCount, candOverflow, t, first + i, __float_as_uint(ta.w), __float_as_uint(tb.w));
                                else candidate_insert<kShadowCandidates>(gbvh, cand, candCount, candOverflow, t, first + i, __float_as_uint(ta.w), __float_as_uint(tb.w));
                                continue;
                            }
                            uint32_t inst = __float_as_uint(ta.w), prim = __float_as_uint(tb.w);
                            const bool ok = OPQ || !lower.have || key_less(lower.t, lower.inst, lower.prim, t, inst, prim);
                            const bool take = ok && (!best.valid || key_less(t, inst, prim, best.t, best.inst, best.prim));
                            best.t = take ? t : best.t; best.u = take ? u : best.u; best.v = take ? v : best.v;
                            best.inst = take ? inst : best.inst; best.prim = take ? prim : best.prim; best.tri = take ? first + i : best.tri;
                            best.opaque = take ? (__float_as_uint(tc.w) & 7u) : best.opaque;
                            best.valid = best.valid || take;
                            tlim = take ? t : tlim;
                        }
                    }
                    cur = (blocked || sp == 0) ? kTraversalDone : stack.pop(--sp);
                }
                if (ANYHIT) {
                    if (cur == kTraversalDone) {
                        HRT_PHASE(PH_ANY_FINISH);
                        const uint32_t id = a.b.sqId[slot];
                        uint32_t code = blocked ? kVisBlocked : kVisClear;
                        if (!blocked && candCount > 0) {
                            uint2* out = a.b.sqCand + (size_t)id * kShadowCandidates;
                            for (int k = 0; k < candCount; ++k) { float ct; uint32_t ctri; cand.key(k, ct, ctri); out[k] = make_uint2(__float_as_uint(ct), ctri); }
                            code = kVisCandidates | ((uint32_t)candCount << 8) | (candOverflow ? 1u << 16 : 0u);
                        }
                        a.b.shVis[id] = code;
                        active = false;
                    }
                } else if (cur == kTraversalDone) {
                    bool done = true;
                    HRT_PHASE(PH_EXT_FINISH);
                    if (!OPQ && TL != 1 && best.valid && !(best.opaque & 1u)) HRT_PHASE(PH_EXT_CANDIDATE);
                    if (!OPQ && TL != 1 && best.valid && !(best.opaque & 1u) && !candidate_commits(s, best, rng)) {
                        lower.have = true; lower.t = best.t; lower.inst = best.inst; lower.prim = best.prim;
                        best.valid = false; tlim = r.tmax; sp = 0;
                        cur = s.nodeCount == 0 ? s.rootLeaf : 0;
                        if constexpr (TL) tl_world(tl, r);
                        done = false;
                    }
                    if (done) {
                        if (!OPQ && a.hasStochasticAlpha && rng != rng0) { float4 d = rayD[slot]; d.w = __uint_as_float(rng); rayD[slot] = d; }
                        a.b.hit[slot] = make_float4(best.t, best.u, best.v, __uint_as_float(best.valid ? (best.tri | ((best.opaque >> 1) << 29)) : 0xFFFFFFFFu));
                        if constexpr (TL) a.b.hitInst[slot] = best.inst;
                        active = false;
                    }
                }
            }
        }
    }
    if (!ANYHIT) block_count_add(&a.counters->closestRays, 0, nRays);
    if (PRIMARY) { __syncthreads(); block_count_add(&a.counters->closestRays, 2, nRays); }
}

struct WfTraceArgs {
    SceneView scene; const HrptRay* rays; HrptRayHit* hits; uint64_t count;
    int32_t* spill; uint32_t refillMin, nodeLoopMin;
    bool quantised;
};
constexpr uint32_t kTraceChunkShift = 8;
template <bool LDS_BVH, int DEPTH, int W, bool SHADOW, bool TL = false>
__global__ __launch_bounds__(kBlock) __attribute__((amdgpu_waves_per_eu(SHADOW ? 1 : (TL ? kWavesExtendTwoLevel : (LDS_BVH ? kWavesExtendLds : kWavesExtendGlobal))))) void wf_trace_rays(WfTraceArgs a)
{
    static_assert(!TL || (!LDS_BVH && W == 4), "two-level structure: global 4-wide trees (every instance opaque: a shadow ray ends at its first hit)");
    static_assert(W != kQuantisedTree || (!LDS_BVH && !TL), "quantised nodes: flat tree in global memory");
    extern __shared__ __attribute__((aligned(128))) char smem[];
    LdsStack<DEPTH, kExtendLdsStack> stack; LdsBvh<W> lbvh;
    constexpr size_t candBytes = SHADOW ? (size_t)kShadowCandidates * 2 * kBlock * 4 : 0;
    setup_lds<LDS_BVH, DEPTH, W>(smem, a.scene, stack, lbvh, candBytes);
    LdsCandidates cand; cand.base = reinterpret_cast<int32_t*>(smem + (size_t)LdsStack<DEPTH, kExtendLdsStack>::kRows * kBlock * 4) + threadIdx.x;
    if (DEPTH > kExtendLdsStack) { stack.spill = a.spill + blockIdx.x * kBlock + threadIdx.x; stack.spillStride = gridDim.x * kBlock; }
    typename GlobalBvhOf<(TL ? kTwoLevelTree : W)>::type gbvh = GlobalBvhOf<(TL ? kTwoLevelTree : W)>::make(a.scene);
    const SceneView& s = a.scene;
    const uint32_t wavesPerBlock = kBlock / 64;
    const uint32_t gw = uniform(blockIdx.x * wavesPerBlock + (threadIdx.x >> 6)), totalWaves = gridDim.x * wavesPerBlock;
    TlCull tl; tl.inv = mk3(0.0f, 0.0f, 0.0f); tl.noi = tl.inv; tl.noiF = tl.inv; tl.inst = -1;
    const uint64_t numChunks = (a.count + (1u << kTraceChunkShift) - 1) >> kTraceChunkShift;
    const bool emptyScene = s.nodeCount == 0 && s.rootLeaf == 0;

    uint64_t chunk = gw; uint32_t cnt = 0, next = 0; uint64_t chunkBase = 0; bool haveChunk = false;
    auto open_chunk = [&]() {
        haveChunk = chunk < numChunks; next = 0;
        if (haveChunk) { chunkBase = chunk << kTraceChunkShift; const uint64_t left = a.count - chunkBase; cnt = left < (1u << kTraceChunkShift) ? (uint32_t)left : (1u << kTraceChunkShift); }
    };
    open_chunk();
    bool active = false;
    Ray r; r.o = mk3(0.0f, 0.0f, 0.0f); r.d = mk3(0.0f, 0.0f, 1.0f); r.tmin = 0.0f; r.tmax = 1e10f;
    RayShear sh = make_shear(r.d); f3 inv = mk3(0.0f, 0.0f, 0.0f), noi = mk3(0.0f, 0.0f, 0.0f);
    HitKey lower; lower.have = false; lower.t = 0.0f; lower.inst = 0; lower.prim = 0;
    Hit best; best.valid = false; best.t = 0.0f; best.inst = 0; best.prim = 0; best.u = 0.0f; best.v = 0.0f; best.opaque = 0; best.tri = 0;
    int32_t cur = kTraversalDone; int sp = 0; uint64_t slot = 0; uint32_t rng = 0; float tlim = 0.0f;
    bool blocked = false, candOverflow = false, finite = true; int candCount = 0;
    for (;;) {
        if (haveChunk && next >= cnt) { chunk += totalWaves; open_chunk(); }
        const unsigned long long mIdle = __ballot(!active);
        const uint32_t nIdle = (uint32_t)__popcll(mIdle);
        if (haveChunk && (nIdle >= a.refillMin || nIdle == 64u)) {
            const uint32_t idx = next + prefix_rank(mIdle);
            if (!active && idx < cnt) {
                slot = chunkBase + idx;
                const float4* rp = reinterpret_cast<const float4*>(a.rays + slot);
                const float4 q0 = rp[0], q1 = rp[1]; const uint32_t rr = reinterpret_cast<const uint32_t*>(rp + 2)[0];
                const f3 o = mk3(q0.x, q0.y, q0.z), d = mk3(q1.x, q1.y, q1.z);
                finite = d.x == d.x && d.y == d.y && d.z == d.z && o.x == o.x && o.y == o.y && o.z == o.z;
                if (SHADOW) r = shadow_ray(o, d, q1.w);
                else { r.o = o; r.d = d; r.tmin = q0.w; r.tmax = q1.w; }
                rng = rr; blocked = false; candOverflow = false; candCount = 0; lower.have = false; best.valid = false; tlim = r.tmax; sp = 0;
                sh = make_shear(r.d);
                if constexpr (TL) tl_world(tl, r); else { inv = traversal_rcp(r.d); noi = slab_origin_term(r.o, inv); }
                cur = (emptyScene || !finite) ? kTraversalDone : (s.nodeCount == 0 ? s.rootLeaf : 0);
                active = true;
            }
            next += nIdle;
        }
        if (__ballot(active) == 0ull) { if (haveChunk) continue; break; }
        if (active) {
            if constexpr (TL) {
                while (cur >= 0 && cur != kExitBlas) {
                    cur = inner_step(gbvh, cur, tl.noi, tl.noiF, tl.inv, r.tmin, tlim, stack, sp);
                    if ((uint32_t)__popcll(__ballot(cur >= 0 && cur != kExitBlas)) < a.nodeLoopMin) break;
                }
                if (cur == kExitBlas || (cur < 0 && cur != kTraversalDone && tl.inst < 0)) cur = tl_switch(gbvh, cur, tl, r, stack, sp);
                else if (cur < 0 && cur != kTraversalDone) {
                    const GpuInstance& I = s.instances[tl.inst];
                    const uint32_t enc = (uint32_t)(~cur), first = enc >> 2, count = (enc & 3u) + 1u, inst = (uint32_t)tl.inst;
                    for (uint32_t i = 0; i < count; ++i) {
                        float4 ta, tb, tc; gbvh.tri(first + i, ta, tb, tc);
                        f3 p0, p1, p2; tl_world_triangle(I, ta, tb, tc, p0, p1, p2);
                        float t, u, v;
                        const bool hitTri = tri_test(p0, p1, p2, r, sh, t, u, v);
                        if (SHADOW) { if (hitTri) { if (I.flags & 1u) { blocked = true; break; } candCount = 1; } continue; }
                        const uint32_t prim = __float_as_uint(tb.w);
                        const bool ok = !lower.have || key_less(lower.t, lower.inst, lower.prim, t, inst, prim);
                        const bool take = hitTri && ok && (!best.valid || key_less(t, inst, prim, best.t, best.inst, best.prim));
                        best.t = take ? t : best.t; best.u = take ? u : best.u; best.v = take ? v : best.v;
                        best.inst = take ? inst : best.inst; best.prim = take ? prim : best.prim; best.tri = take ? first + i : best.tri;
                        best.valid = best.valid || take; best.opaque = take ? (I.flags & 1u) : best.opaque;
                        tlim = take ? t : tlim;
                    }
                    cur = blocked ? kTraversalDone : stack.pop(--sp);
                }
            } else {
            while (cur >= 0) {
                if (LDS_BVH) cur = inner_step(lbvh, cur, noi, inv, r.tmin, tlim, stack, sp);
                else cur = inner_step(gbvh, cur, noi, inv, r.tmin, tlim, stack, sp);
                if ((uint32_t)__popcll(__ballot(cur >= 0)) < a.nodeLoopMin) break;
            }
            if (cur < 0 && cur != kTraversalDone) {
                const uint32_t enc = (uint32_t)(~cur), first = enc >> 2, count = (enc & 3u) + 1u;
                for (uint32_t i = 0; i < count; ++i) {
                    float4 ta, tb, tc;
                    if (LDS_BVH) lbvh.tri(first + i, ta, tb, tc); else gbvh.tri(first + i, ta, tb, tc);
                    float t, u, v;
                    if (tri_test(mk3(ta.x, ta.y, ta.z), mk3(tb.x, tb.y, tb.z), mk3(tc.x, tc.y, tc.z), r, sh, t, u, v)) {
                        if (SHADOW) {
                            if (__float_as_uint(tc.w) & 1u) { blocked = true; break; }
                            if (LDS_BVH) candidate_insert<kShadowCandidates>(lbvh, cand, candCount, candOverflow, t, first + i, __float_as_uint(ta.w), __float_as_uint(tb.w));
                            else candidate_insert<kShadowCandidates>(gbvh, cand, candCount, candOverflow, t, first + i, __float_as_uint(ta.w), __float_as_uint(tb.w));
                            continue;
                        }
                        const uint32_t inst = __float_as_uint(ta.w), prim = __float_as_uint(tb.w);
                        const bool ok = !lower.have || key_less(lower.t, lower.inst, lower.prim, t, inst, prim);
                        const bool take = ok && (!best.valid || key_less(t, inst, prim, best.t, best.inst, best.prim));
                        best.t = take ? t : best.t; best.u = take ? u : best.u; best.v = take ? v : best.v;
                        best.inst = take ? inst : best.inst; best.prim = take ? prim : best.prim; best.tri = take ? first + i : best.tri;
                        best.opaque = take ? (__float_as_uint(tc.w) & 1u) : best.opaque;
                        best.valid = best.valid || take;
                        tlim = take ? t : tlim;
                    }
                }
                cur = (blocked || sp == 0) ? kTraversalDone : stack.pop(--sp);
            }
            }
            if (cur == kTraversalDone) {
                HrptRayHit out; out.t = 0.0f; out.u = 0.0f; out.v = 0.0f; out.instance = 0; out.primitive = 0; out.hit = 0; out.rng = rng; out.pad = 0;
                bool done = true;
                if (SHADOW) {
                    float vis = 1.0f;
                    if (finite) {
                        if (blocked) vis = 0.0f;
                        else if (candCount > 0) {
                            if constexpr (TL) vis = shadow_retrace_two_level(s, gbvh, r, stack);
                            else if (LDS_BVH) vis = shadow_resolve_candidates(s, lbvh, r, sh, candCount, candOverflow, cand, stack);
                            else vis = shadow_resolve_candidates(s, gbvh, r, sh, candCount, candOverflow, cand, stack);
                        }
                    }
                    out.t = vis; out.hit = vis < 1.0f ? 1u : 0u;
                } else if (best.valid && !best.opaque && !candidate_commits(s, best, rng)) {
                    lower.have = true; lower.t = best.t; lower.inst = best.inst; lower.prim = best.prim;
                    best.valid = false; tlim = r.tmax; sp = 0;
                    cur = s.nodeCount == 0 ? s.rootLeaf : 0;
                    if constexpr (TL) tl_world(tl, r);
                    done = false;
                } else if (best.valid) { out.t = best.t; out.u = best.u; out.v = best.v; out.instance = best.inst; out.primitive = best.prim; out.hit = 1u; out.rng = rng; }
                if (done) {
                    out.rng = rng;
                    float4* hp = reinterpret_cast<float4*>(a.hits + slot);
                    hp[0] = make_float4(out.t, out.u, out.v, __uint_as_float(out.instance));
                    hp[1] = make_float4(__uint_as_float(out.primitive), __uint_as_float(out.hit), __uint_as_float(out.rng), 0.0f);
                    active = false;
                }
            }
        }
    }
}

template <int MAXL>
struct NeeBuf { float ux[MAXL], uy[MAXL]; uint32_t light[MAXL]; };

HRT_DEV LdsShadeTables copy_shade_tables(char* dst, const WfArgs& a)
{
    const SceneView& s = a.scene;
    const uint32_t nA = s.triCount * (uint32_t)(sizeof(GpuTriAttr) / 16), nI = a.shadeInstances * (uint32_t)(sizeof(GpuInstShade) / 16);
    const uint32_t nM = a.shadeMaterials * (uint32_t)(sizeof(HrptMaterialConstants) / 4);
    float4* const dA = reinterpret_cast<float4*>(dst); float4* const dI = dA + nA; uint32_t* const dM = reinterpret_cast<uint32_t*>(dI + nI);
    const float4* const sA = reinterpret_cast<const float4*>(s.attrs); const float4* const sI = reinterpret_cast<const float4*>(s.instShade);
    const uint32_t* const sM = reinterpret_cast<const uint32_t*>(s.materials);
    for (uint32_t i = threadIdx.x; i < nA; i += kBlock) dA[i] = sA[i];
    for (uint32_t i = threadIdx.x; i < nI; i += kBlock) dI[i] = sI[i];
    for (uint32_t i = threadIdx.x; i < nM; i += kBlock) dM[i] = sM[i];
    LdsShadeTables t;
    t.attrs = (uint32_t)(uintptr_t)(LdsShadeTables::LdsPtr)dst; t.instShade = t.attrs + nA * 16u; t.materials = t.instShade + nI * 16u;
    return t;
}


template <int MAXL, bool SIMPLE, bool PRIMARY, bool LDS_TABLES>
HRT_DEV void shade_paths(const WfArgs& a, const HrptPathTracerConstants& cb, uint32_t parity, int bounce, int lastBounce)
{
    static_assert(!PRIMARY || SIMPLE, "no raygen pass: SIMPLE scenes only");
    static_assert(!LDS_TABLES || SIMPLE, "tables in LDS: behind the ring of the SIMPLE variants");
    const uint32_t wavesPerBlock = kBlock / 64, lane = lane_id();
    const uint32_t gw = uniform(blockIdx.x * wavesPerBlock + (threadIdx.x >> 6)), totalWaves = gridDim.x * wavesPerBlock;
    const uint32_t in = parity, out = parity ^ 1u;
    const SceneView& s = a.scene;
    extern __shared__ __attribute__((aligned(16))) char shadeSmem[];
    constexpr uint32_t kRing = kShadeRing, kRingFields = kShadeRingFields;
    float* const ring = reinterpret_cast<float*>(shadeSmem) + (size_t)uniform(threadIdx.x >> 6) * kRing * kRingFields;
    LdsShadeTables ldsTables; ldsTables.attrs = ldsTables.instShade = ldsTables.materials = 0u;
    if constexpr (LDS_TABLES) { ldsTables = copy_shade_tables(shadeSmem + kShadeRingBytes, a); __syncthreads(); }
    const GlobalShadeTables globalTables{ s };
    auto shade_hit = [&](PathState& ps, const Hit& h, SurfaceCarry& carry, auto&& emit) {
        if constexpr (LDS_TABLES) return shade_surface_a<!SIMPLE, !SIMPLE, SIMPLE>(s, ldsTables, cb, ps, h, carry, emit);
        else return shade_surface_a<!SIMPLE, !SIMPLE, SIMPLE>(s, globalTables, cb, ps, h, carry, emit);
    };
    uint32_t ringHead = 0, pending = 0;
    unsigned int nEntriesOut = 0, nRadiance = 0;
    constexpr bool SORT = !SIMPLE;
    const uint32_t segSize = a.segSize;
    uint16_t* const permBase = reinterpret_cast<uint16_t*>(shadeSmem) + (size_t)uniform(threadIdx.x >> 6) * segSize * 2;
    uint8_t* const keys = reinterpret_cast<uint8_t*>(shadeSmem) + (size_t)wavesPerBlock * segSize * 4 + (size_t)uniform(threadIdx.x >> 6) * segSize;
    uint32_t permSel = 0;
    bool permuted = false, permutedB = false;
    auto sort_segment = [&](uint32_t base, uint32_t n, uint16_t* perm) -> bool {
        HRT_PHASE(PH_SHADE_SORT);
        uint32_t c0 = 0, c1 = 0, c2 = 0;
        for (uint32_t b = 0; b < n; b += 64) {
            const uint32_t e = b + lane; uint32_t k = 4u;
            if (e < n) { k = __float_as_uint(a.b.hit[base + e].w) >> 29; k = k > 3u ? 3u : k; keys[e] = (uint8_t)k; }
            c0 += (uint32_t)__popcll(__ballot(k == 0u)); c1 += (uint32_t)__popcll(__ballot(k == 1u)); c2 += (uint32_t)__popcll(__ballot(k == 2u));
        }
        const uint32_t c3 = n - c0 - c1 - c2;
        if (c0 == n || c1 == n || c2 == n || c3 == n) return false;
        __builtin_amdgcn_fence(__ATOMIC_SEQ_CST, "wavefront");
        uint32_t b0 = 0, b1 = c0, b2 = c0 + c1, b3 = c0 + c1 + c2;
        for (uint32_t b = 0; b < n; b += 64) {
            const uint32_t e = b + lane; const uint32_t k = e < n ? keys[e] : 4u;
            const unsigned long long m0 = __ballot(k == 0u), m1 = __ballot(k == 1u), m2 = __ballot(k == 2u), m3 = __ballot(k == 3u);
            if (k == 0u) perm[b0 + prefix_rank(m0)] = (uint16_t)e;
            if (k == 1u) perm[b1 + prefix_rank(m1)] = (uint16_t)e;
            if (k == 2u) perm[b2 + prefix_rank(m2)] = (uint16_t)e;
            if (k == 3u) perm[b3 + prefix_rank(m3)] = (uint16_t)e;
            b0 += (uint32_t)__popcll(m0); b1 += (uint32_t)__popcll(m1); b2 += (uint32_t)__popcll(m2); b3 += (uint32_t)__popcll(m3);
        }
        __builtin_amdgcn_fence(__ATOMIC_SEQ_CST, "wavefront");
        return true;
    };
    {
        uint32_t seg = gw, cnt = 0, segBase = 0, next = 0, outCount = 0, shCount = 0;
        bool haveSeg = false;
        auto open_segment = [&]() {
            haveSeg = false; cnt = 0; next = 0; outCount = 0; shCount = 0;
            for (; seg < a.numSegments; seg += totalWaves) {
                cnt = uniform(PRIMARY ? path_count(a, in, seg) : a.b.pathCnt[in][seg]);
                if (cnt) { segBase = seg * a.segSize; haveSeg = true; break; }
                if (lane == 0) { a.b.pathCnt[out][seg] = 0; a.b.shadowCnt[seg] = 0; }
            }
            if (SORT && a.sortShade && haveSeg) permuted = sort_segment(segBase, cnt, permBase + permSel * segSize);
        };
        open_segment();
        while (haveSeg) {
            const uint32_t takeA = cnt - next < 64u ? cnt - next : 64u;
            const uint32_t segA = seg, baseA = segBase, nextA = next;
            const bool endsA = nextA + takeA >= cnt;
            uint32_t takeB = 0, segB = 0, baseB = 0, cntB = 0;
            if (endsA && takeA < 64u) {
                uint32_t probe = seg + totalWaves;
                for (; probe < a.numSegments; probe += totalWaves) {
                    cntB = uniform(PRIMARY ? path_count(a, in, probe) : a.b.pathCnt[in][probe]);
                    if (cntB) break;
                    if (lane == 0) { a.b.pathCnt[out][probe] = 0; a.b.shadowCnt[probe] = 0; }
                }
                if (probe < a.numSegments) {
                    segB = probe; baseB = probe * a.segSize; takeB = cntB < 64u - takeA ? cntB : 64u - takeA;
                    if (SORT && a.sortShade) permutedB = sort_segment(baseB, cntB, permBase + (permSel ^ 1u) * segSize);
                } else segB = probe;
            }
            const bool inA = lane < takeA;
            uint32_t outCountB = 0, shCountB = 0;
            bool valid = lane < takeA + takeB, alive = false, wantDefer = false, wantRadiance = false;
            LobeDraw ld; ld.spec = false; ld.specProb = 0.0f; ld.root = 0.0f; ld.sp = 0.0f; ld.cp = 0.0f;
            uint32_t nNee = 0, smp = 0, slotIn = 0;
            PathState ps; f3 neeT = mk3(0.0f, 0.0f, 0.0f);
            constexpr bool STREAMED = MAXL == 0;
            NeeBuf<(STREAMED ? 1 : MAXL)> nee; SurfaceCarry carry;
            if (valid) {
                HRT_PHASE(PH_SHADE_ITER);
                uint32_t slot = inA ? baseA + ((SORT && permuted) ? (uint32_t)permBase[permSel * segSize + nextA + lane] : nextA + lane)
                                    : baseB + ((SORT && permutedB) ? (uint32_t)permBase[(permSel ^ 1u) * segSize + (lane - takeA)] : lane - takeA);
                slotIn = slot;
                float4 o, d, t;
                if constexpr (PRIMARY) {
                    const PrimaryArgs& pr = *a.primaryArgs;
                    o = make_float4(pr.cam[0], pr.cam[1], pr.cam[2], 0.0f); d = a.b.rayD[in][slot];
                    t = make_float4(1.0f, 1.0f, 1.0f, __uint_as_float(slot));
                } else { o = a.b.rayO[in][slot]; d = a.b.rayD[in][slot]; t = a.b.thr[in][slot]; }
                float4 ha = a.b.hit[slot]; uint32_t tri = __float_as_uint(ha.w);
                const bool noPath = PRIMARY && tri == kNoPathRecord;
                if (tri < kNoPathRecord) tri &= 0x1FFFFFFFu;
                ps.ray.o = mk3(o.x, o.y, o.z); ps.ray.d = mk3(d.x, d.y, d.z); ps.ray.tmin = o.w; ps.ray.tmax = 1e10f;
                ps.rng = __float_as_uint(d.w);
                ps.throughput = mk3(t.x, t.y, t.z); smp = __float_as_uint(t.w);
                ps.radiance = mk3(0.0f, 0.0f, 0.0f);
                if (!SIMPLE && a.hasMedium) {
                    float4 m0 = a.b.med0[in][slot], m1 = a.b.med1[in][slot];
                    ps.sigmaA = mk3(m0.x, m0.y, m0.z); ps.interiorIOR = m0.w; ps.sigmaS = mk3(m1.x, m1.y, m1.z); ps.inVolume = m1.w != 0.0f;
                } else { ps.sigmaA = mk3(0.0f, 0.0f, 0.0f); ps.sigmaS = mk3(0.0f, 0.0f, 0.0f); ps.interiorIOR = 1.0f; ps.inVolume = false; }
// ... 59 lines not shown
            const unsigned long long msA = __ballot(nNee > 0 && inA), msB = __ballot(nNee > 0 && !inA);
            if (SIMPLE && MAXL == 1 && a.slimShadow && nNee > 0) {
                uint32_t e = inA ? baseA + shCount + prefix_rank(msA) : baseB + prefix_rank(msB);
                a.b.sh0[e] = make_float4(carry.worldPos.x, carry.worldPos.y, carry.worldPos.z, __uint_as_float(slotIn));
                a.b.sh1[e] = make_float4(carry.N.x, carry.N.y, carry.N.z, __uint_as_float(carry.material));
            } else if (nNee > 0) {
                uint32_t e = inA ? baseA + shCount + prefix_rank(msA) : baseB + prefix_rank(msB);
                a.b.sh0[e] = make_float4(carry.worldPos.x, carry.worldPos.y, carry.worldPos.z, __uint_as_float(smp));
                a.b.sh1[e] = make_float4(carry.N.x, carry.N.y, carry.N.z, carry.roughness);
                a.b.sh2[e] = make_float4(carry.V.x, carry.V.y, carry.V.z, carry.metallic);
                a.b.sh3[e] = make_float4(carry.baseColor.x, carry.baseColor.y, carry.baseColor.z, carry.ior);
                a.b.sh4[e] = make_float4(neeT.x, neeT.y, neeT.z, __uint_as_float(nNee));
                if (STREAMED) {
                    const f3 sunDir = mk3(cb.m_SunDirection[0], cb.m_SunDirection[1], cb.m_SunDirection[2]);
                    uint32_t rng = carry.rngBeforeLights, j = 0;
                    for (uint32_t i = 0; i < cb.m_LightCount; ++i) {
                        HrptGPULight l = load_light(s, i);
                        float ux, uy;
                        if (nee_draw<false>(l, carry.N, carry.worldPos, sunDir, rng, ux, uy)) a.b.shL[(size_t)e * a.maxLights + j++] = make_float4(ux, uy, __uint_as_float(i), 0.0f);
                    }
                } else {
#pragma unroll
                    for (int j = 0; j < (STREAMED ? 1 : MAXL); ++j)
                        if ((uint32_t)j < nNee) a.b.shL[(size_t)e * a.maxLights + j] = make_float4(nee.ux[j], nee.uy[j], __uint_as_float(nee.light[j]), 0.0f);
                }
            }
            outCount += (uint32_t)__popcll(mA); shCount += (uint32_t)__popcll(msA);
            outCountB = (uint32_t)__popcll(mB); shCountB = (uint32_t)__popcll(msB);
            nEntriesOut += (unsigned int)(__popcll(msA) + __popcll(msB));
            if (SIMPLE) {
                const unsigned long long md = __ballot(wantDefer);
                const uint32_t nNew = (uint32_t)__popcll(md);
                bool parked = false;
                for (int round = 0; round < 2 && !parked; ++round) {
                parked = pending + nNew <= kRing;
                if (parked && wantDefer) {
                    float* e = ring + ((ringHead + pending + prefix_rank(md)) & (kRing - 1u));
                    e[0 * kRing] = carry.N.x; e[1 * kRing] = carry.N.y; e[2 * kRing] = carry.N.z;
                    e[3 * kRing] = carry.V.x; e[4 * kRing] = carry.V.y; e[5 * kRing] = carry.V.z;
                    e[6 * kRing] = carry.F0.x; e[7 * kRing] = carry.F0.y; e[8 * kRing] = carry.F0.z;
                    e[9 * kRing] = carry.roughness; e[10 * kRing] = ld.root; e[11 * kRing] = ld.sp; e[12 * kRing] = ld.cp; e[13 * kRing] = ld.specProb;
                    e[14 * kRing] = carry.worldPos.x; e[15 * kRing] = carry.worldPos.y; e[16 * kRing] = carry.worldPos.z;
                    e[17 * kRing] = ps.throughput.x; e[18 * kRing] = ps.throughput.y; e[19 * kRing] = ps.throughput.z;
                    e[20 * kRing] = __uint_as_float(ps.rng); e[21 * kRing] = __uint_as_float(smp); e[22 * kRing] = inA ? 1.0f : 0.0f;
                }
                if (parked) pending += nNew;
                __builtin_amdgcn_fence(__ATOMIC_SEQ_CST, "wavefront");
                while (pending >= 64u || ((endsA || !parked) && pending)) {
                    const uint32_t n = pending < 64u ? pending : 64u;
                    bool alive2 = false, tagA = true; PathState q; uint32_t smp2 = 0;
                    if (lane < n) {
                        const float* e = ring + ((ringHead + lane) & (kRing - 1u));
                        f3 N = mk3(e[0 * kRing], e[1 * kRing], e[2 * kRing]), V = mk3(e[3 * kRing], e[4 * kRing], e[5 * kRing]), F0 = mk3(e[6 * kRing], e[7 * kRing], e[8 * kRing]);
                        LobeDraw d2; d2.spec = true; d2.root = e[10 * kRing]; d2.sp = e[11 * kRing]; d2.cp = e[12 * kRing]; d2.specProb = e[13 * kRing];
                        f3 wp = mk3(e[14 * kRing], e[15 * kRing], e[16 * kRing]);
                        q.throughput = mk3(e[17 * kRing], e[18 * kRing], e[19 * kRing]); q.rng = __float_as_uint(e[20 * kRing]); smp2 = __float_as_uint(e[21 * kRing]);
                        tagA = e[22 * kRing] != 0.0f;
                        alive2 = lobe_specular(q, wp, N, V, F0, e[9 * kRing], d2);
                    }
                    const unsigned long long m2A = __ballot(alive2 && tagA), m2B = __ballot(alive2 && !tagA);
                    if (alive2) {
                        uint32_t o = tagA ? baseA + outCount + prefix_rank(m2A) : baseB + outCountB + prefix_rank(m2B);
                        a.b.rayO[out][o] = make_float4(q.ray.o.x, q.ray.o.y, q.ray.o.z, q.ray.tmin);
                        a.b.rayD[out][o] = make_float4(q.ray.d.x, q.ray.d.y, q.ray.d.z, __uint_as_float(q.rng));
                        a.b.thr[out][o] = make_float4(q.throughput.x, q.throughput.y, q.throughput.z, __uint_as_float(smp2));
                    }
                    outCount += (uint32_t)__popcll(m2A); outCountB += (uint32_t)__popcll(m2B);
                    ringHead = (ringHead + n) & (kRing - 1u); pending -= n;
                    __builtin_amdgcn_fence(__ATOMIC_SEQ_CST, "wavefront");
                }
                }
            }
            if (!endsA) next = nextA + takeA;
            else {
                if (lane == 0) { a.b.pathCnt[out][segA] = outCount; a.b.shadowCnt[segA] = shCount; }
                if (takeB) {
                    seg = segB; segBase = baseB; cnt = cntB; next = takeB;
                    outCount = outCountB; shCount = shCountB;
                    haveSeg = true;
                    if (SORT) { permSel ^= 1u; permuted = permutedB; permutedB = false; }
                    if (next >= cnt) {
                        if (lane == 0) { a.b.pathCnt[out][seg] = outCount; a.b.shadowCnt[seg] = shCount; }
                        seg += totalWaves; open_segment();
                    }
                } else if (takeA < 64u) { seg = segB; haveSeg = false; }
                else { seg += totalWaves; open_segment(); }
            }
        }
    }
    block_count_add_uniform<2>(a.counters, { 3, 5 }, { nEntriesOut, nRadiance });
}
template <int MAXL, bool SIMPLE, bool PRIMARY = false>
__global__ __launch_bounds__(kBlock) __attribute__((amdgpu_waves_per_eu(kWavesShade, kWavesShade))) void wf_shade(WfArgs a, HrptPathTracerConstants cb, uint32_t parity, int bounce, int lastBounce)
{
    shade_paths<MAXL, SIMPLE, PRIMARY, false>(a, cb, parity, bounce, lastBounce);
}
template <int MAXL, bool SIMPLE, bool PRIMARY = false>
__global__ __launch_bounds__(kBlock) __attribute__((amdgpu_waves_per_eu(kWavesShade, kWavesShade))) void wf_shade_lt(WfArgs a, HrptPathTracerConstants cb, uint32_t parity, int bounce, int lastBounce)
{
    shade_paths<MAXL, SIMPLE, PRIMARY, true>(a, cb, parity, bounce, lastBounce);
}

template <bool DIRONLY>
__global__ __launch_bounds__(kBlock) void wf_shadow_rays(WfArgs a, HrptPathTracerConstants cb)
{
    const SceneView& s = a.scene;
    const f3 sunDir = mk3(cb.m_SunDirection[0], cb.m_SunDirection[1], cb.m_SunDirection[2]);
    const uint32_t wavesPerBlock = kBlock / 64, lane = lane_id();
    const uint32_t gw = uniform(blockIdx.x * wavesPerBlock + (threadIdx.x >> 6)), totalWaves = gridDim.x * wavesPerBlock;
    for (uint32_t seg = gw; seg < a.numSegments; seg += totalWaves) {
        const uint32_t cnt = uniform(a.b.shadowCnt[seg]), segBase = seg * a.segSize, items = cnt * a.maxLights;
        uint32_t outCount = 0;
        for (uint32_t i0 = 0; i0 < items; i0 += 64) {
            const uint32_t i = i0 + lane;
            bool valid = false; Ray ray; uint32_t id = 0;
            if (i < items) {
                HRT_PHASE(PH_SHADOW_RAYS_ITEM);
                const uint32_t el = i / a.maxLights, j = i - el * a.maxLights, e = segBase + el;
                id = e * a.maxLights + j;
                float4 h4 = a.b.sh4[e];
                if (j < __float_as_uint(h4.w)) {
                    float4 h0 = a.b.sh0[e], h1 = a.b.sh1[e], ls = a.b.shL[(size_t)e * a.maxLights + j];
                    HrptGPULight l = load_light(s, __float_as_uint(ls.z));
                    f3 L; float maxDist;
                    if (nee_direction<DIRONLY>(l, mk3(h1.x, h1.y, h1.z), mk3(h0.x, h0.y, h0.z), sunDir, cb.m_CosSunAngularRadius, ls.x, ls.y, L, maxDist)) {
                        ray = shadow_ray(mk3(h0.x, h0.y, h0.z), L, maxDist);
                        valid = true;
                    }
                }
                if (!valid) a.b.shVis[id] = kVisNoRay;
            }
            const unsigned long long m = __ballot(valid);
            if (valid) {
                const uint32_t o = segBase * a.maxLights + outCount + prefix_rank(m);
                a.b.sqO[o] = make_float4(ray.o.x, ray.o.y, ray.o.z, ray.tmin);
                a.b.sqD[o] = make_float4(ray.d.x, ray.d.y, ray.d.z, ray.tmax);
                a.b.sqId[o] = id;
            }
            outCount += (uint32_t)__popcll(m);
        }
        if (lane == 0) a.b.sqCnt[seg] = outCount;
    }
}

template <bool LDS_BVH, int DEPTH, int W, bool DIRONLY, int MODE, int TL = 0>
__global__ __launch_bounds__(kBlock) __attribute__((amdgpu_waves_per_eu(MODE == 2 && TL == 0 ? 4 : ((MODE == 1 || TL != 0) ? 3 : 1)))) void wf_shadow(WfArgs a, HrptPathTracerConstants cb, int bounce)
{
    static_assert(!TL || (!LDS_BVH && W == 4 && (MODE == kShadowOpaque || MODE == kShadowSlim)), "two-level structure: opaque any-hit query over the global tree");
    static_assert(W != kQuantisedTree || (!LDS_BVH && !TL), "quantised nodes: flat tree in global memory");
    constexpr bool NONOPAQUE = MODE == kShadowBuffered || MODE == kShadowResolve;
    constexpr bool SLIM = MODE == kShadowSlim;
    constexpr int kLdsMax = MODE == kShadowResolve ? kExtendLdsStack : kShadowLdsStack;
    extern __shared__ __attribute__((aligned(128))) char smem[];
    LdsStack<DEPTH, kLdsMax> stack; LdsBvh<W> lbvh;
    constexpr size_t candBytes = MODE == kShadowBuffered ? (size_t)kShadowCandidates * 2 * kBlock * 4 : 0;
    setup_lds<LDS_BVH, DEPTH, W>(smem, a.scene, stack, lbvh, candBytes);
    if (DEPTH > kLdsMax) { stack.spill = a.spill[1] + blockIdx.x * kBlock + threadIdx.x; stack.spillStride = gridDim.x * kBlock; }
    LdsCandidates cand; cand.base = reinterpret_cast<int32_t*>(smem + (size_t)LdsStack<DEPTH, kLdsMax>::kRows * kBlock * 4) + threadIdx.x;
    LdsCandidates3 cand3; cand3.base = cand.base;
    typename GlobalBvhOf<(TL ? kTwoLevelTree : W)>::type gbvh = GlobalBvhOf<(TL ? kTwoLevelTree : W)>::make(a.scene);
    const SceneView& s = a.scene;
    const f3 sunDir = mk3(cb.m_SunDirection[0], cb.m_SunDirection[1], cb.m_SunDirection[2]);
    const float sunIntensity = s.lights[0].m_Intensity;

    const uint32_t wavesPerBlock = kBlock / 64, lane = lane_id();
    const uint32_t gw = uniform(blockIdx.x * wavesPerBlock + (threadIdx.x >> 6)), totalWaves = gridDim.x * wavesPerBlock;
    unsigned int nRays = 0, nSamples = 0, nRadiance = 0, nSkipped16 = 0;
    auto process = [&](uint32_t e) {
                HRT_PHASE(PH_SHADOW_ENTRY);
                if (SLIM) {
                    const float4 h0 = a.b.sh0[e], h1 = a.b.sh1[e];
                    const uint32_t slot = __float_as_uint(h0.w);
                    const float4 rd = a.b.rayD[a.shadowParity][slot];
                    const f3 origin = mk3(h0.x, h0.y, h0.z), N = mk3(h1.x, h1.y, h1.z);
                    uint32_t rng = __float_as_uint(rd.w);
                    const float ux = hrt_rng_next(&rng), uy = hrt_rng_next(&rng);
                    ++nSamples;
                    HrptGPULight l = load_light(s, 0u);
                    f3 L; float maxDist;
                    if (!nee_direction<true>(l, N, origin, sunDir, cb.m_CosSunAngularRadius, ux, uy, L, maxDist)) return;
                    float shadow;
                    if (LDS_BVH) shadow = shadow_query<true>(s, lbvh, origin, L, maxDist, stack);
                    else if constexpr (TL == 2) shadow = shadow_query_two_level_buffered<kTwoLevelCandidates>(s, gbvh, shadow_ray(origin, L, maxDist), stack, cand3);
                    else shadow = shadow_query<true>(s, gbvh, origin, L, maxDist, stack);
                    ++nRays;
                    if (shadow != 0.0f) {
                        const float4 th = a.primary ? make_float4(1.0f, 1.0f, 1.0f, __uint_as_float(slot)) : a.b.thr[a.shadowParity][slot];
                        if (a.primary) ++nSkipped16;
                        const HrptMaterialConstants& mat = s.materials[__float_as_uint(h1.w)];
                        f3 dif, spec;
                        nee_contribution<true>(s, l, nee_lighting(N, mk3(-rd.x, -rd.y, -rd.z), mk3(mat.m_BaseColor), hrt_max(mat.m_RoughnessMetallic[0], 0.04f),
                                                                  mat.m_RoughnessMetallic[1], mat.m_IOR), origin, sunDir, sunIntensity, L, dif, spec);
                        f3 totalDiffuse = mk3(0.0f, 0.0f, 0.0f) + dif * shadow, totalSpecular = mk3(0.0f, 0.0f, 0.0f);
                        if (bounce == 0) totalSpecular = totalSpecular + spec * shadow;
                        const f3 dsum = totalDiffuse + (bounce == 0 ? totalSpecular : mk3(0.0f, 0.0f, 0.0f));
                        if (dsum.x != 0.0f || dsum.y != 0.0f || dsum.z != 0.0f) {
                            const f3 term = mk3(th.x, th.y, th.z) * dsum;
                            const uint32_t smp = __float_as_uint(th.w);
                            float4 r = a.b.radiance[smp];
                            r.x = r.x + term.x; r.y = r.y + term.y; r.z = r.z + term.z;
                            a.b.radiance[smp] = r;
                            ++nRadiance;
                        }
                    }
                    return;
                }
                float4 h0 = a.b.sh0[e], h1 = a.b.sh1[e], h4 = a.b.sh4[e];
                f3 origin = mk3(h0.x, h0.y, h0.z), N = mk3(h1.x, h1.y, h1.z), T = mk3(h4.x, h4.y, h4.z);
                uint32_t smp = __float_as_uint(h0.w), n = __float_as_uint(h4.w);
                nSamples += n;
                f3 totalDiffuse = mk3(0.0f, 0.0f, 0.0f), totalSpecular = mk3(0.0f, 0.0f, 0.0f);
                float4 ls0 = make_float4(0.0f, 0.0f, 0.0f, 0.0f);
                if (MODE != kShadowResolve && n) ls0 = a.b.shL[(size_t)e * a.maxLights];
                for (uint32_t j = 0; j < n; ++j) {
                    HRT_PHASE(PH_SHADOW_SAMPLE);
                    uint32_t vis = kVisCandidates;
                    if (MODE == kShadowResolve) {
                        vis = a.b.shVis[e * a.maxLights + j];
                        if (vis == kVisNoRay) continue;
                        if (vis == kVisBlocked) { ++nRays; continue; }
                    }
                    float4 ls = ls0;
                    if (MODE == kShadowResolve || j) ls = a.b.shL[(size_t)e * a.maxLights + j];
                    HrptGPULight l = load_light(s, __float_as_uint(ls.z));
                    f3 L; float maxDist;
                    if (!nee_direction<DIRONLY>(l, N, origin, sunDir, cb.m_CosSunAngularRadius, ls.x, ls.y, L, maxDist)) continue;
                    float shadow;
                    HRT_PHASE(PH_SHADOW_QUERY);
                    if (MODE == kShadowResolve) {
                        if (vis == kVisClear) shadow = 1.0f;
                        else {
                            Ray sr = shadow_ray(origin, L, maxDist);
                            GlobalCandidates gc; gc.base = a.b.sqCand + (size_t)(e * a.maxLights + j) * kShadowCandidates;
                            const int cnt = (int)((vis >> 8) & 0xFFu); const bool ovf = (vis >> 16) & 1u;
                            if (LDS_BVH) shadow = shadow_resolve_candidates(s, lbvh, sr, make_shear(sr.d), cnt, ovf, gc, stack);
                            else shadow = shadow_resolve_candidates(s, gbvh, sr, make_shear(sr.d), cnt, ovf, gc, stack);
                        }
                    } else if (MODE == kShadowBuffered) {
                        if (LDS_BVH) shadow = shadow_query_buffered<kShadowCandidates>(s, lbvh, origin, L, maxDist, stack, cand);
                        else shadow = shadow_query_buffered<kShadowCandidates>(s, gbvh, origin, L, maxDist, stack, cand);
                    } else {
                        if (LDS_BVH) shadow = shadow_query<true>(s, lbvh, origin, L, maxDist, stack);
                        else if constexpr (TL == 2) shadow = shadow_query_two_level_buffered<kTwoLevelCandidates>(s, gbvh, shadow_ray(origin, L, maxDist), stack, cand3);
                    else shadow = shadow_query<true>(s, gbvh, origin, L, maxDist, stack);
                    }
                    ++nRays;
                    if (shadow != 0.0f) {
                        HRT_PHASE(PH_SHADOW_CONTRIB);
                        float4 h2 = a.b.sh2[e], h3 = a.b.sh3[e];
                        f3 dif, spec;
                        nee_contribution<DIRONLY>(s, l, nee_lighting(N, mk3(h2.x, h2.y, h2.z), mk3(h3.x, h3.y, h3.z), h1.w, h2.w, h3.w), origin, sunDir,
                                                  sunIntensity, L, dif, spec);
                        totalDiffuse = totalDiffuse + dif * shadow;
                        if (bounce == 0) totalSpecular = totalSpecular + spec * shadow;
                    }
                }
                f3 dsum = totalDiffuse + (bounce == 0 ? totalSpecular : mk3(0.0f, 0.0f, 0.0f));
                if (dsum.x != 0.0f || dsum.y != 0.0f || dsum.z != 0.0f) {
                    f3 term = T * dsum;
                    float4 r = a.b.radiance[smp];
                    r.x = r.x + term.x; r.y = r.y + term.y; r.z = r.z + term.z;
                    a.b.radiance[smp] = r;
                    ++nRadiance;
                }
    };
    if (NONOPAQUE) {
        uint32_t seg = gw, cnt = 0, segBase = 0, next = 0; bool haveSeg = false;
        auto open_segment = [&]() {
            haveSeg = false; cnt = 0; next = 0;
            for (; seg < a.numSegments; seg += totalWaves) {
                cnt = uniform(a.b.shadowCnt[seg]);
                if (cnt) { segBase = seg * a.segSize; haveSeg = true; break; }
            }
        };
        open_segment();
        while (haveSeg) {
            uint32_t e = 0xFFFFFFFFu, filled = 0;
            while (filled < 64u && haveSeg) {
                uint32_t take = cnt - next < 64u - filled ? cnt - next : 64u - filled;
                if (lane >= filled && lane < filled + take) e = segBase + next + (lane - filled);
                next += take; filled += take;
                if (next >= cnt) { seg += totalWaves; open_segment(); }
            }
            if (e != 0xFFFFFFFFu) process(e);
        }
    } else {
        for (uint32_t seg = gw; seg < a.numSegments; seg += totalWaves) {
            const uint32_t cnt = uniform(a.b.shadowCnt[seg]), segBase = seg * a.segSize;
            for (uint32_t base = 0; base < cnt; base += 64) {
                uint32_t i = base + lane;
                if (i < cnt) process(segBase + i);
            }
        }
    }
    block_count_add(&a.counters->closestRays, 1, nRays);
    __syncthreads();
    block_count_add(&a.counters->closestRays, 4, nSamples);
    __syncthreads();
    block_count_add(&a.counters->closestRays, 6, nRadiance);
    if (SLIM && a.primary) { __syncthreads(); block_count_add(&a.counters->closestRays, 7, nSkipped16); }
}

__global__ __launch_bounds__(kBlock) void wf_resolve(WfArgs a, float4* __restrict__ accumulation, float4* __restrict__ output, uint32_t firstIndex)
{
    uint32_t p = blockIdx.x * blockDim.x + threadIdx.x;
    uint32_t stride = gridDim.x * blockDim.x;
    for (; p < a.pixelsPadded; p += stride) {
        uint32_t tile = p >> 6, within = p & 63u;
        uint32_t tcol, trow; tile_position(a, tile, tcol, trow);
        uint32_t px = a.rect.column_x(tcol) + (within & 7u), py = a.rect.y0 + trow * 8u + (within >> 3);
        if (px >= a.rect.x1 || py >= a.rect.y1) continue;
        size_t idx = (size_t)py * a.imageWidth + px;
        float4 acc = make_float4(0.0f, 0.0f, 0.0f, 0.0f);
        for (uint32_t k = 0; k < a.spp; ++k) {
            float4 r = a.b.radiance[(size_t)k * a.pixelsPadded + p];
            float4 cur = make_float4(r.x, r.y, r.z, 1.0f);
            if (firstIndex + k > 0) {
                float4 prev = (k == 0) ? accumulation[idx] : acc;
                cur.x += prev.x; cur.y += prev.y; cur.z += prev.z; cur.w += prev.w;
            }
            acc = cur;
        }
        accumulation[idx] = acc;
        output[idx] = make_float4(acc.x / acc.w, acc.y / acc.w, acc.z / acc.w, 1.0f);
    }
}

__global__ __launch_bounds__(kBlock) void wf_gbuffer(WfArgs a, HrptPathTracerConstants cb, GBufferPlanes g, uint32_t planeMask)
{
    const uint32_t wavesPerBlock = kBlock / 64, lane = lane_id();
    const uint32_t gw = uniform(blockIdx.x * wavesPerBlock + (threadIdx.x >> 6)), totalWaves = gridDim.x * wavesPerBlock;
    const SceneView& s = a.scene;
    for (uint32_t seg = gw; seg < a.numSegments; seg += totalWaves) {
        const uint32_t cnt = uniform(a.b.pathCnt[0][seg]), segBase = seg * a.segSize;
        for (uint32_t base = 0; base < cnt; base += 64) {
            if (base + lane >= cnt) continue;
            const uint32_t slot = segBase + base + lane;
            const float4 o = a.b.rayO[0][slot], d = a.b.rayD[0][slot], ha = a.b.hit[slot];
            const uint32_t smp = reinterpret_cast<const uint32_t*>(a.b.thr[0] + slot)[3];
            const uint32_t tile = smp >> 6, within = smp & 63u;
            const bool columnMajor = a.rect.stripeCount > 1u;
            const uint32_t den = columnMajor ? a.tilesY : a.tilesX, quo = tile / den, rem = tile - quo * den;
            const uint32_t tcol = columnMajor ? quo : rem, trow = columnMajor ? rem : quo;
            const uint32_t px = a.rect.column_x(tcol) + (within & 7u), py = a.rect.y0 + trow * 8u + (within >> 3);
            uint32_t tri = __float_as_uint(ha.w);
            float4 texel[kGbPlanes];
            if (tri != 0xFFFFFFFFu) {
                tri &= 0x1FFFFFFFu;
                Ray ray; ray.o = mk3(o.x, o.y, o.z); ray.d = mk3(d.x, d.y, d.z); ray.tmin = o.w; ray.tmax = 1e10f;
                Hit h; h.valid = true; h.t = ha.x; h.u = ha.y; h.v = ha.z; h.tri = tri; h.prim = 0; h.inst = s.instances ? a.b.hitInst[slot] : 0u; h.opaque = 1;
                gbuffer_texels(s, cb, ray, h, texel);
            } else gbuffer_miss(texel);
            gbuffer_store(g, planeMask, (size_t)py * a.imageWidth + px, texel);
        }
    }
}

template <bool PLANES>
__global__ __launch_bounds__(kBlock) __attribute__((amdgpu_waves_per_eu(4))) void wf_gbuffer_motion(WfArgs a, HrptPathTracerConstants cb, GBufferPlanes g, uint32_t planeMask, MotionArgs m)
{
    const uint32_t wavesPerBlock = kBlock / 64, lane = lane_id();
    const uint32_t gw = uniform(blockIdx.x * wavesPerBlock + (threadIdx.x >> 6)), totalWaves = gridDim.x * wavesPerBlock;
    const SceneView& s = a.scene;
    for (uint32_t seg = gw; seg < a.numSegments; seg += totalWaves) {
        const uint32_t cnt = uniform(a.b.pathCnt[0][seg]), segBase = seg * a.segSize;
        for (uint32_t base = 0; base < cnt; base += 64) {
            if (base + lane >= cnt) continue;
            const uint32_t slot = segBase + base + lane;
            const float4 o = a.b.rayO[0][slot], d = a.b.rayD[0][slot], ha = a.b.hit[slot];
            const uint32_t smp = reinterpret_cast<const uint32_t*>(a.b.thr[0] + slot)[3];
            const uint32_t tile = smp >> 6, within = smp & 63u;
            const bool columnMajor = a.rect.stripeCount > 1u;
            const uint32_t den = columnMajor ? a.tilesY : a.tilesX, quo = tile / den, rem = tile - quo * den;
            const uint32_t tcol = columnMajor ? quo : rem, trow = columnMajor ? rem : quo;
            const uint32_t px = a.rect.column_x(tcol) + (within & 7u), py = a.rect.y0 + trow * 8u + (within >> 3);
            const size_t idx = (size_t)py * a.imageWidth + px;
            uint32_t tri = __float_as_uint(ha.w);
            float4 texel[kGbPlanes];
            float4 motion = make_float4(0.0f, 0.0f, 0.0f, 0.0f);
            if (tri != 0xFFFFFFFFu) {
                tri &= 0x1FFFFFFFu;
                Hit h; h.valid = true; h.t = ha.x; h.u = ha.y; h.v = ha.z; h.tri = tri; h.prim = 0; h.inst = s.instances ? a.b.hitInst[slot] : 0u; h.opaque = 1;
                const MotionTri mt = motion_gather(s, m, h);
                if constexpr (PLANES) {
                    Ray ray; ray.o = mk3(o.x, o.y, o.z); ray.d = mk3(d.x, d.y, d.z); ray.tmin = o.w; ray.tmax = 1e10f;
                    gbuffer_texels(s, cb, ray, h, texel);
                }
                motion = motion_texel(cb.m_View, m, mt, h.u, h.v);
            } else if constexpr (PLANES) gbuffer_miss(texel);
// ... 459 lines not shown
```

Baseline: 27170 Mrays/s.

## Store LDS triangles as per-axis rows and pick shear axes by address offset

Triangles copied into LDS are now stored as records with x, y and z components in separate rows, so the ray's shear permutation turns into per-ray byte offsets. The triangle test then loads the permuted components straight from LDS instead of loading whole float4s and selecting components with runtime kx/ky/kz branches or selects. Instance, prim and flag words are read from LDS only when they are needed. This cuts ALU select work in the watertight triangle test, at the cost of more scalar LDS loads and a reshuffle during LDS setup.

Result: no change. 27340 Mrays/s (median of 2 runs) (+0.6%).

```diff
diff --git a/hobbyrenderer_amd/csrc/pt_device.h b/hobbyrenderer_amd/csrc/pt_device.h
--- a/hobbyrenderer_amd/csrc/pt_device.h
+++ b/hobbyrenderer_amd/csrc/pt_device.h
@@ -2,9 +2,11 @@
 
 #include <hip/hip_runtime.h>
 #include <stdint.h>
+#include <type_traits>
 
 #include "../../include/hobbyrt_pt.h"
 #include "../../include/hobbyrt/detmath.h"
+#include "../../include/hobbyrt/tri_forms.h"
 #include "../../include/hobbyrt/srgb_table.h"
 
 #define HRT_DEV __device__ __forceinline__
@@ -124,21 +126,8 @@
 struct Hit { float t; uint32_t inst, prim; float u, v; uint32_t opaque; uint32_t tri; bool valid; };
 struct HitKey { float t; uint32_t inst, prim; bool have; };
 
-struct RayShear { int kx, ky, kz; float Sx, Sy, Sz; };
-
-HRT_DEV RayShear make_shear(f3 d)
-{
-    RayShear s;
-    int kz = 0;
-    if (hrt_abs(d.y) > hrt_abs(comp(d, kz))) kz = 1;
-    if (hrt_abs(d.z) > hrt_abs(comp(d, kz))) kz = 2;
-    int kx = (kz + 1) % 3, ky = (kx + 1) % 3;
-    if (comp(d, kz) < 0.0f) { int t = kx; kx = ky; ky = t; }
-    s.kx = kx; s.ky = ky; s.kz = kz;
-    float dz = comp(d, kz);
-    s.Sx = comp(d, kx) / dz; s.Sy = comp(d, ky) / dz; s.Sz = 1.0f / dz;
-    return s;
-}
+typedef HrtTriShear RayShear;
+HRT_DEV RayShear make_shear(f3 d) { return hrt_tri_shear(d.x, d.y, d.z); }
 HRT_DEV bool key_less(float t, uint32_t inst, uint32_t prim, float t2, uint32_t inst2, uint32_t prim2)
 {
     if (t < t2) return true;
@@ -150,23 +139,20 @@
 HRT_DEV bool tri_test(f3 p0, f3 p1, f3 p2, const Ray& r, const RayShear& s, float& t, float& u, float& v)
 {
     f3 A = p0 - r.o, B = p1 - r.o, C = p2 - r.o;
-    float Akz = comp(A, s.kz), Bkz = comp(B, s.kz), Ckz = comp(C, s.kz);
-    float Ax = comp(A, s.kx) - s.Sx * Akz, Ay = comp(A, s.ky) - s.Sy * Akz;
-    float Bx = comp(B, s.kx) - s.Sx * Bkz, By = comp(B, s.ky) - s.Sy * Bkz;
-    float Cx = comp(C, s.kx) - s.Sx * Ckz, Cy = comp(C, s.ky) - s.Sy * Ckz;
-    float U = Cx * By - Cy * Bx;
-    float V = Ax * Cy - Ay * Cx;
-    float W = Bx * Ay - By * Ax;
-    if ((U < 0.0f || V < 0.0f || W < 0.0f) && (U > 0.0f || V > 0.0f || W > 0.0f)) return false;
-    float det = (U + V) + W;
-    if (det == 0.0f) return false;
-    float Az = s.Sz * Akz, Bz = s.Sz * Bkz, Cz = s.Sz * Ckz;
-    float T = (U * Az + V * Bz) + W * Cz;
-    float rcp = 1.0f / det;
-    float tt = T * rcp;
-    if (!(tt > r.tmin && tt < r.tmax)) return false;
-    t = tt; u = V * rcp; v = W * rcp;
-    return true;
+    return hrt_tri_core(comp(A, s.kx), comp(A, s.ky), comp(A, s.kz), comp(B, s.kx), comp(B, s.ky), comp(B, s.kz),
+                        comp(C, s.kx), comp(C, s.ky), comp(C, s.kz), s.Sx, s.Sy, s.Sz, r.tmin, r.tmax, &t, &u, &v) != 0;
+}
+typedef HrtTriRows LdsRayShear;
+constexpr uint32_t kLdsTriBytes = 48u, kLdsTriInst = 36u, kLdsTriPrim = 40u, kLdsTriFlags = 44u;
+typedef __attribute__((address_space(3))) const float* LdsFloatPtr;
+typedef __attribute__((address_space(3))) const uint32_t* LdsWordPtr;
+HRT_DEV LdsRayShear make_lds_shear(f3 o, f3 d) { return hrt_tri_rows(o.x, o.y, o.z, d.x, d.y, d.z); }
+HRT_DEV uint32_t lds_word(uint32_t address) { return *(LdsWordPtr)(uintptr_t)address; }
+HRT_DEV bool tri_test_lds(uint32_t record, const LdsRayShear& s, float tmin, float tmax, float& t, float& u, float& v)
+{
+    const LdsFloatPtr x = (LdsFloatPtr)(uintptr_t)(record + s.rx), y = (LdsFloatPtr)(uintptr_t)(record + s.ry), z = (LdsFloatPtr)(uintptr_t)(record + s.rz);
+    return hrt_tri_core(x[0] - s.ox, y[0] - s.oy, z[0] - s.oz, x[1] - s.ox, y[1] - s.oy, z[1] - s.oz,
+                        x[2] - s.ox, y[2] - s.oy, z[2] - s.oz, s.Sx, s.Sy, s.Sz, tmin, tmax, &t, &u, &v) != 0;
 }
 
 struct GlobalBvh {
@@ -208,6 +194,46 @@
 };
 template <class BVH, class = void> struct IsQuantised { static constexpr bool value = false; };
 template <class BVH> struct IsQuantised<BVH, decltype((void)BVH::kQuantised)> { static constexpr bool value = true; };
+template <class BVH, class = void> struct IsLds { static constexpr bool value = false; };
+template <class BVH> struct IsLds<BVH, std::enable_if_t<BVH::kLds>> { static constexpr bool value = true; };
+template <class BVH, class = void> struct IsRows { static constexpr bool value = false; };
+template <class BVH> struct IsRows<BVH, std::enable_if_t<BVH::kLds && BVH::kRows>> { static constexpr bool value = true; };
+template <class BVH> struct ShearOf { typedef std::conditional_t<IsRows<BVH>::value, LdsRayShear, RayShear> type; };
+struct TriWords { uint32_t i, p, f; HRT_DEV uint32_t inst() const { return i; } HRT_DEV uint32_t prim() const { return p; } HRT_DEV uint32_t flags() const { return f; } };
+struct LdsTriWords {
+    uint32_t record;
+    HRT_DEV uint32_t inst() const { return lds_word(record + kLdsTriInst); }
+    HRT_DEV uint32_t prim() const { return lds_word(record + kLdsTriPrim); }
+    HRT_DEV uint32_t flags() const { return lds_word(record + kLdsTriFlags); }
+};
+template <class BVH> struct TriWordsOf { typedef std::conditional_t<IsRows<BVH>::value, LdsTriWords, TriWords> type; };
+template <class BVH>
+HRT_DEV typename ShearOf<BVH>::type ray_shear(const BVH&, const Ray& r)
+{
+    if constexpr (IsRows<BVH>::value) return make_lds_shear(r.o, r.d); else return make_shear(r.d);
+}
+template <class BVH>
+HRT_DEV bool leaf_test(const BVH& bvh, uint32_t i, const Ray& r, const typename ShearOf<BVH>::type& sh, float& t, float& u, float& v, typename TriWordsOf<BVH>::type& w)
+{
+    if constexpr (IsRows<BVH>::value) { w.record = bvh.record(i); return tri_test_lds(w.record, sh, r.tmin, r.tmax, t, u, v); }
+    else if constexpr (IsLds<BVH>::value) {
+        typedef __attribute__((address_space(3))) const char* LdsBytePtr;
+        const float4* q = reinterpret_cast<const float4*>((const char*)(LdsBytePtr)(uintptr_t)bvh.record(i));
+        const float4 a = q[0], b = q[1], c = q[2];
+        w.i = __float_as_uint(c.y); w.p = __float_as_uint(c.z); w.f = __float_as_uint(c.w);
+        return tri_test(mk3(a.x, a.w, b.z), mk3(a.y, b.x, b.w), mk3(a.z, b.y, c.x), r, sh, t, u, v);
+    } else {
+        float4 a, b, c; bvh.tri(i, a, b, c);
+        w.i = __float_as_uint(a.w); w.p = __float_as_uint(b.w); w.f = __float_as_uint(c.w);
+        return tri_test(mk3(a.x, a.y, a.z), mk3(b.x, b.y, b.z), mk3(c.x, c.y, c.z), r, sh, t, u, v);
+    }
+}
+template <class BVH>
+HRT_DEV void tri_key(const BVH& bvh, uint32_t i, uint32_t& inst, uint32_t& prim)
+{
+    if constexpr (IsLds<BVH>::value) { const uint32_t rec = bvh.record(i); inst = lds_word(rec + kLdsTriInst); prim = lds_word(rec + kLdsTriPrim); }
+    else { float4 a, b, c; bvh.tri(i, a, b, c); inst = __float_as_uint(a.w); prim = __float_as_uint(b.w); }
+}
 
 HRT_DEV f3 slab_origin_term(f3 o, f3 inv) { return mk3(-(o.x * inv.x), -(o.y * inv.y), -(o.z * inv.z)); }
 HRT_DEV bool slab(float4 bmin, float4 bmax, f3 noi, f3 inv, float t0, float t1, float& tnear)
@@ -322,7 +348,7 @@
 {
     Hit best; best.valid = false; best.t = r.tmax; best.inst = 0; best.prim = 0; best.u = 0; best.v = 0; best.opaque = 0; best.tri = 0;
     if (!(r.d.x == r.d.x && r.d.y == r.d.y && r.d.z == r.d.z)) return best;
-    RayShear sh = make_shear(r.d);
+    const typename ShearOf<BVH>::type sh = ray_shear(bvh, r);
     f3 inv = traversal_rcp(r.d), noi = slab_origin_term(r.o, inv);
     int sp = 0;
     int32_t cur;
@@ -339,15 +365,15 @@
             uint32_t enc = (uint32_t)(~cur);
             uint32_t first = enc >> 2, count = (enc & 3u) + 1u;
             for (uint32_t i = 0; i < count; ++i) {
-                float4 a, b, c; bvh.tri(first + i, a, b, c);
+                typename TriWordsOf<BVH>::type w;
                 float t, u, v;
-                if (tri_test(mk3(a.x, a.y, a.z), mk3(b.x, b.y, b.z), mk3(c.x, c.y, c.z), r, sh, t, u, v)) {
-                    uint32_t inst = __float_as_uint(a.w), prim = __float_as_uint(b.w);
+                if (leaf_test(bvh, first + i, r, sh, t, u, v, w)) {
+                    uint32_t inst = w.inst(), prim = w.prim();
                     bool ok = !lower.have || key_less(lower.t, lower.inst, lower.prim, t, inst, prim);
                     const bool take = ok && (!best.valid || key_less(t, inst, prim, best.t, best.inst, best.prim));
                     best.t = take ? t : best.t; best.u = take ? u : best.u; best.v = take ? v : best.v;
                     best.inst = take ? inst : best.inst; best.prim = take ? prim : best.prim; best.tri = take ? first + i : best.tri;
-                    best.opaque = take ? (__float_as_uint(c.w) & 1u) : best.opaque;
+                    best.opaque = take ? (w.flags() & 1u) : best.opaque;
                     best.valid = best.valid || take;
                     tlim = take ? t : tlim;
                 }
@@ -364,7 +390,7 @@
 {
     sawNonOpaque = false;
     if (!(r.d.x == r.d.x && r.d.y == r.d.y && r.d.z == r.d.z)) return false;
-    RayShear sh = make_shear(r.d);
+    const typename ShearOf<BVH>::type sh = ray_shear(bvh, r);
     f3 inv = traversal_rcp(r.d), noi = slab_origin_term(r.o, inv);
     int sp = 0; int32_t cur;
     if (nodeCount == 0) { if (rootLeaf == 0) return false; cur = rootLeaf; }
@@ -379,10 +405,10 @@
             uint32_t enc = (uint32_t)(~cur);
             uint32_t first = enc >> 2, count = (enc & 3u) + 1u;
             for (uint32_t i = 0; i < count; ++i) {
-                float4 a, b, c; bvh.tri(first + i, a, b, c);
+                typename TriWordsOf<BVH>::type w;
                 float t, u, v;
-                if (tri_test(mk3(a.x, a.y, a.z), mk3(b.x, b.y, b.z), mk3(c.x, c.y, c.z), r, sh, t, u, v)) {
-                    if (__float_as_uint(c.w) & 1u) return true;
+                if (leaf_test(bvh, first + i, r, sh, t, u, v, w)) {
+                    if (w.flags() & 1u) return true;
                     sawNonOpaque = true;
                 }
             }
diff --git a/hobbyrenderer_amd/csrc/pt_path.h b/hobbyrenderer_amd/csrc/pt_path.h
--- a/hobbyrenderer_amd/csrc/pt_path.h
+++ b/hobbyrenderer_amd/csrc/pt_path.h
@@ -277,16 +277,16 @@
     int pos = count;
     if (count == K) {
         float lt; uint32_t ltri; cand.key(K - 1, lt, ltri);
-        float4 la, lb, lc; bvh.tri(ltri, la, lb, lc);
+        uint32_t linst, lprim; tri_key(bvh, ltri, linst, lprim);
         overflow = true;
-        if (!key_less(t, inst, prim, lt, __float_as_uint(la.w), __float_as_uint(lb.w))) return;
+        if (!key_less(t, inst, prim, lt, linst, lprim)) return;
         pos = K - 1;
     } else ++count;
     while (pos > 0) {
         float pt; uint32_t ptri; cand.key(pos - 1, pt, ptri);
         bool less;
         if (t != pt) less = t < pt;
-        else { float4 pa, pb, pc; bvh.tri(ptri, pa, pb, pc); less = key_less(t, inst, prim, pt, __float_as_uint(pa.w), __float_as_uint(pb.w)); }
+        else { uint32_t pinst, pprim; tri_key(bvh, ptri, pinst, pprim); less = key_less(t, inst, prim, pt, pinst, pprim); }
         if (!less) break;
         cand.move(pos, pos - 1);
         --pos;
@@ -294,22 +294,21 @@
     cand.set(pos, t, tri);
 }
 template <class BVH, class STACK, class CAND>
-HRT_DEV float shadow_resolve_candidates(const SceneView& s, const BVH& bvh, const Ray& ray, const RayShear& sh, int count, bool overflow, const CAND& cand, STACK& stack)
+HRT_DEV float shadow_resolve_candidates(const SceneView& s, const BVH& bvh, const Ray& ray, const typename ShearOf<BVH>::type& sh, int count, bool overflow, const CAND& cand, STACK& stack)
 {
     if (count == 0) return 1.0f;
     ShadowState st; st.transmission = 1.0f; st.inVolume = false; st.inVolumeStartT = 0.0f; st.sigmaT = mk3(0.0f, 0.0f, 0.0f);
     float lastT = 0.0f; uint32_t lastTri = 0;
     for (int k = 0; k < count; ++k) {
         float t; uint32_t tri; cand.key(k, t, tri);
-        float4 a, b, c; bvh.tri(tri, a, b, c);
+        typename TriWordsOf<BVH>::type w;
         float t2, u, v;
-        tri_test(mk3(a.x, a.y, a.z), mk3(b.x, b.y, b.z), mk3(c.x, c.y, c.z), ray, sh, t2, u, v);
+        leaf_test(bvh, tri, ray, sh, t2, u, v, w);
         if (shadow_candidate(s, ray, t, tri, u, v, st)) return 0.0f;
         lastT = t; lastTri = tri;
     }
     if (overflow) {
-        float4 la, lb, lc; bvh.tri(lastTri, la, lb, lc);
-        HitKey lower; lower.have = true; lower.t = lastT; lower.inst = __float_as_uint(la.w); lower.prim = __float_as_uint(lb.w);
+        HitKey lower; lower.have = true; lower.t = lastT; tri_key(bvh, lastTri, lower.inst, lower.prim);
         for (;;) {
             Hit h = closest_any(bvh, s.rootLeaf, s.nodeCount, ray, lower, stack);
             if (!h.valid) break;
@@ -325,7 +324,7 @@
 {
     Ray ray = shadow_ray(worldPos, L, maxDist);
     if (!(ray.d.x == ray.d.x && ray.d.y == ray.d.y && ray.d.z == ray.d.z)) return 1.0f;
-    RayShear sh = make_shear(ray.d);
+    const typename ShearOf<BVH>::type sh = ray_shear(bvh, ray);
     f3 inv = traversal_rcp(ray.d), noi = slab_origin_term(ray.o, inv);
     int sp = 0, count = 0; bool overflow = false;
     int32_t cur;
@@ -340,11 +339,11 @@
         uint32_t enc = (uint32_t)(~cur);
         uint32_t first = enc >> 2, n = (enc & 3u) + 1u;
         for (uint32_t i = 0; i < n; ++i) {
-            float4 a, b, c; bvh.tri(first + i, a, b, c);
+            typename TriWordsOf<BVH>::type w;
             float t, u, v;
-            if (!tri_test(mk3(a.x, a.y, a.z), mk3(b.x, b.y, b.z), mk3(c.x, c.y, c.z), ray, sh, t, u, v)) continue;
-            if (__float_as_uint(c.w) & 1u) return 0.0f;
-            candidate_insert<K>(bvh, cand, count, overflow, t, first + i, __float_as_uint(a.w), __float_as_uint(b.w));
+            if (!leaf_test(bvh, first + i, ray, sh, t, u, v, w)) continue;
+            if (w.flags() & 1u) return 0.0f;
+            candidate_insert<K>(bvh, cand, count, overflow, t, first + i, w.inst(), w.prim());
         }
         if (sp == 0) break;
         cur = stack.pop(--sp);
diff --git a/hobbyrenderer_amd/csrc/pt_wavefront.hip b/hobbyrenderer_amd/csrc/pt_wavefront.hip
--- a/hobbyrenderer_amd/csrc/pt_wavefront.hip
+++ b/hobbyrenderer_amd/csrc/pt_wavefront.hip
@@ -135,16 +135,17 @@
     const uint2* base;
     HRT_DEV void key(int k, float& t, uint32_t& tri) const { uint2 v = base[k]; t = __uint_as_float(v.x); tri = v.y; }
 };
-template <int W>
+template <int W, bool ROWS = true>
 struct LdsBvh {
-    static constexpr int kWidth = W == 5 ? 4 : W; static constexpr bool kTwoLevel = false; static constexpr bool kLds = true;
+    static constexpr int kWidth = W == 5 ? 4 : W; static constexpr bool kTwoLevel = false; static constexpr bool kLds = true; static constexpr bool kRows = ROWS;
+    typedef __attribute__((address_space(3))) const char* LdsPtr;
     const float4* nodes; const float4* tris;
     HRT_DEV void node(int i, float4& a, float4& b, float4& c, float4& d) const { const float4* p = nodes + 4 * i; a = p[0]; b = p[1]; c = p[2]; d = p[3]; }
-    HRT_DEV void tri(uint32_t i, float4& a, float4& b, float4& c) const { const float4* p = tris + 3 * i; a = p[0]; b = p[1]; c = p[2]; }
-    typedef __attribute__((address_space(3))) const char* LdsPtr;
+    HRT_DEV uint32_t record(uint32_t i) const { return (uint32_t)(uintptr_t)(LdsPtr) reinterpret_cast<const char*>(tris) + i * kLdsTriBytes; }
     HRT_DEV uint32_t rowoff(int i, uint32_t byteOffset) const { return (uint32_t)(uintptr_t)(LdsPtr) reinterpret_cast<const char*>(nodes) + (uint32_t)i * kLdsNode4Stride + byteOffset; }
     HRT_DEV float4 load(uint32_t off) const { return *reinterpret_cast<const float4*>((const char*)(LdsPtr)(uintptr_t)off); }
 };
+template <bool LDS, class L, class G> HRT_DEV const std::conditional_t<LDS, L, G>& pick_bvh(const L& l, const G& g) { if constexpr (LDS) return l; else return g; }
 template <int W> struct GlobalBvhOf;
 template <> struct GlobalBvhOf<2> { using type = GlobalBvh; static HRT_DEV GlobalBvh make(const SceneView& s) { GlobalBvh g; g.nodes = s.nodes; g.tris = s.tris; return g; } };
 constexpr int kTwoLevelTree = 44;
@@ -153,8 +154,8 @@
 constexpr int kQuantisedTree = 5;
 template <> struct GlobalBvhOf<kQuantisedTree> { using type = GlobalBvhQ; static HRT_DEV GlobalBvhQ make(const SceneView& s) { GlobalBvhQ g; g.nodes = s.nodesQ; g.tris = s.tris; return g; } };
 
-template <bool LDS_BVH, int DEPTH, int W, int LDSMAX>
-HRT_DEV void setup_lds(char* smem, const SceneView& s, LdsStack<DEPTH, LDSMAX>& stack, LdsBvh<W>& lbvh, size_t extraBytes = 0)
+template <bool LDS_BVH, int DEPTH, int W, int LDSMAX, bool ROWS>
+HRT_DEV void setup_lds(char* smem, const SceneView& s, LdsStack<DEPTH, LDSMAX>& stack, LdsBvh<W, ROWS>& lbvh, size_t extraBytes = 0)
 {
     stack.base = reinterpret_cast<int32_t*>(smem) + threadIdx.x;
     stack.spill = nullptr; stack.spillStride = 0;
@@ -166,7 +167,13 @@
         uint32_t nNdst = nN;
         if (W == 2 || kLdsNode4Stride == 128u) { for (uint32_t i = threadIdx.x; i < nN; i += kBlock) dst[i] = srcN[i]; }
         else { nNdst = s.node4Count * (kLdsNode4Stride / 16u); for (uint32_t i = threadIdx.x; i < nN; i += kBlock) dst[(i >> 3) * (kLdsNode4Stride / 16u) + (i & 7u)] = srcN[i]; }
-        for (uint32_t i = threadIdx.x; i < nT; i += kBlock) dst[nNdst + i] = srcT[i];
+        float* dstT = reinterpret_cast<float*>(dst + nNdst);
+        for (uint32_t i = threadIdx.x; i < nT; i += kBlock) {
+            const float4 p = srcT[i];
+            const uint32_t q = i / 3u, j = i - q * 3u;
+            float* rec = dstT + q * 12u + j;
+            rec[0] = p.x; rec[3] = p.y; rec[6] = p.z; rec[9] = p.w;
+        }
         lbvh.nodes = dst; lbvh.tris = dst + nNdst;
         __syncthreads();
     }
@@ -278,6 +285,9 @@
 #define HRPT_WAVES_EXTEND_LDS_OPAQUE 6
 #endif
 constexpr int kWavesExtendLdsOpaque = HRPT_WAVES_EXTEND_LDS_OPAQUE;
+#ifndef HRPT_EXTEND_LEAN
+#define HRPT_EXTEND_LEAN 1
+#endif
 static_assert(sizeof(GpuTriAttr) == kTriAttrBytes && sizeof(GpuInstShade) == kInstShadeBytes && sizeof(HrptMaterialConstants) == kMaterialBytes, "pt_wavefront_plan.h shade_table_bytes");
 constexpr uint32_t kNoPathRecord = 0xFFFFFFFEu;
 
@@ -289,12 +299,16 @@
     static_assert(!PRIMARY || !ANYHIT, "primary rays are closest-hit rays");
     static_assert(W != kQuantisedTree || (!LDS_BVH && !TL), "quantised nodes: flat tree in global memory");
     extern __shared__ __attribute__((aligned(128))) char smem[];
-    LdsStack<DEPTH, kExtendLdsStack> stack; LdsBvh<W> lbvh;
+    LdsStack<DEPTH, kExtendLdsStack> stack; LdsBvh<W, (OPQ || !PRIMARY)> lbvh;
     constexpr size_t candBytes = ANYHIT ? (size_t)kShadowCandidates * 2 * kBlock * 4 : 0;
     setup_lds<LDS_BVH, DEPTH, W>(smem, a.scene, stack, lbvh, candBytes);
     LdsCandidates cand; cand.base = reinterpret_cast<int32_t*>(smem + (size_t)LdsStack<DEPTH, kExtendLdsStack>::kRows * kBlock * 4) + threadIdx.x;
     if (DEPTH > kExtendLdsStack) { stack.spill = a.spill[ANYHIT ? 1 : 0] + blockIdx.x * kBlock + threadIdx.x; stack.spillStride = gridDim.x * kBlock; }
     typename GlobalBvhOf<(TL ? kTwoLevelTree : W)>::type gbvh = GlobalBvhOf<(TL ? kTwoLevelTree : W)>::make(a.scene);
+    typedef std::conditional_t<LDS_BVH, decltype(lbvh), typename GlobalBvhOf<(TL ? kTwoLevelTree : W)>::type> Bvh;
+    const Bvh& bvh = pick_bvh<LDS_BVH>(lbvh, gbvh);
+    constexpr bool LEAN = LDS_BVH && OPQ && HRPT_EXTEND_LEAN;
+    constexpr uint32_t kNoTriangle = 0xFFFFFFFFu;
     const SceneView& s = a.scene;
 
     const uint32_t wavesPerBlock = kBlock / 64;
@@ -319,11 +333,12 @@
         open_segment();
         bool active = false;
         Ray r; r.o = mk3(0.0f, 0.0f, 0.0f); r.d = mk3(0.0f, 0.0f, 1.0f); r.tmin = 0.0f; r.tmax = 1e10f;
-        RayShear sh = make_shear(r.d); f3 inv = mk3(0.0f, 0.0f, 0.0f), noi = mk3(0.0f, 0.0f, 0.0f);
+        typename ShearOf<Bvh>::type sh = ray_shear(bvh, r); f3 inv = mk3(0.0f, 0.0f, 0.0f), noi = mk3(0.0f, 0.0f, 0.0f);
         TlCull tl; tl.inv = inv; tl.noi = noi; tl.noiF = noi; tl.inst = -1;
         HitKey lower; lower.have = false; lower.t = 0.0f; lower.inst = 0; lower.prim = 0;
         Hit best; best.valid = false; best.t = 0.0f; best.inst = 0; best.prim = 0; best.u = 0.0f; best.v = 0.0f; best.opaque = 0; best.tri = 0;
         int32_t cur = kTraversalDone; int sp = 0; uint32_t slot = 0, rng = 0, rng0 = 0; float tlim = 0.0f;
+        float& limit = LEAN ? best.t : tlim;
         bool blocked = false, candOverflow = false; int candCount = 0;
         for (;;) {
             if (haveSeg && next >= cnt && (a.streamSegments || __ballot(active) == 0ull)) { seg += totalWaves; open_segment(); }
@@ -351,8 +366,9 @@
                     blocked = false; candOverflow = false; candCount = 0;
                     lower.have = false;
                     best.valid = false; tlim = r.tmax; sp = 0;
+                    if constexpr (LEAN) { best.t = r.tmax; best.tri = kNoTriangle; }
                     bool finite = (r.d.x == r.d.x && r.d.y == r.d.y && r.d.z == r.d.z);
-                    sh = make_shear(r.d);
+                    sh = ray_shear(bvh, r);
                     if constexpr (TL) tl_world(tl, r); else { inv = traversal_rcp(r.d); noi = slab_origin_term(r.o, inv); }
                     cur = (emptyScene || !finite) ? kTraversalDone : (s.nodeCount == 0 ? s.rootLeaf : 0);
                     active = true; ++nRays;
@@ -390,8 +406,7 @@
                 } else {
                 while (cur >= 0) {
                     HRT_PHASE(ANYHIT ? PH_ANY_NODE : PH_EXT_NODE);
-                    if (LDS_BVH) cur = inner_step(lbvh, cur, noi, inv, r.tmin, tlim, stack, sp);
-                    else cur = inner_step(gbvh, cur, noi, inv, r.tmin, tlim, stack, sp);
+                    cur = inner_step(bvh, cur, noi, inv, r.tmin, limit, stack, sp);
                     if ((uint32_t)__popcll(__ballot(cur >= 0)) < a.nodeLoopMin) break;
                 }
                 }
@@ -401,22 +416,29 @@
                     HRT_PHASE(ANYHIT ? PH_ANY_LEAF : PH_EXT_LEAF);
                     for (uint32_t i = 0; i < count; ++i) {
                         HRT_PHASE(ANYHIT ? PH_ANY_TRI : PH_EXT_TRI);
-                        float4 ta, tb, tc;
-                        if (LDS_BVH) lbvh.tri(first + i, ta, tb, tc); else gbvh.tri(first + i, ta, tb, tc);
+                        typename TriWordsOf<Bvh>::type w;
                         float t, u, v;
-                        if (tri_test(mk3(ta.x, ta.y, ta.z), mk3(tb.x, tb.y, tb.z), mk3(tc.x, tc.y, tc.z), r, sh, t, u, v)) {
+                        if (leaf_test(bvh, first + i, r, sh, t, u, v, w)) {
                             if (ANYHIT) {
-                                if (__float_as_uint(tc.w) & 1u) { blocked = true; break; }
-                                if (LDS_BVH) candidate_insert<kShadowCandidates>(lbvh, cand, candCount, candOverflow, t, first + i, __float_as_uint(ta.w), __float_as_uint(tb.w));
-                                else candidate_insert<kShadowCandidates>(gbvh, cand, candCount, candOverflow, t, first + i, __float_as_uint(ta.w), __float_as_uint(tb.w));
+                                if (w.flags() & 1u) { blocked = true; break; }
+                                candidate_insert<kShadowCandidates>(bvh, cand, candCount, candOverflow, t, first + i, w.inst(), w.prim());
                                 continue;
                             }
-                            uint32_t inst = __float_as_uint(ta.w), prim = __float_as_uint(tb.w);
+                            if constexpr (LEAN) {
+                                bool take = t < best.t;
+                                if (t == best.t && best.tri != kNoTriangle) {
+                                    uint32_t binst, bprim; tri_key(bvh, best.tri, binst, bprim);
+                                    take = key_less(t, w.inst(), w.prim(), best.t, binst, bprim);
+                                }
+                                best.t = take ? t : best.t; best.u = take ? u : best.u; best.v = take ? v : best.v; best.tri = take ? first + i : best.tri;
+                                continue;
+                            }
+                            uint32_t inst = w.inst(), prim = w.prim();
                             const bool ok = OPQ || !lower.have || key_less(lower.t, lower.inst, lower.prim, t, inst, prim);
                             const bool take = ok && (!best.valid || key_less(t, inst, prim, best.t, best.inst, best.prim));
                             best.t = take ? t : best.t; best.u = take ? u : best.u; best.v = take ? v : best.v;
                             best.inst = take ? inst : best.inst; best.prim = take ? prim : best.prim; best.tri = take ? first + i : best.tri;
-                            best.opaque = take ? (__float_as_uint(tc.w) & 7u) : best.opaque;
+                            best.opaque = take ? (w.flags() & 7u) : best.opaque;
                             best.valid = best.valid || take;
                             tlim = take ? t : tlim;
                         }
@@ -449,6 +471,11 @@
                     }
                     if (done) {
                         if (!OPQ && a.hasStochasticAlpha && rng != rng0) { float4 d = rayD[slot]; d.w = __uint_as_float(rng); rayD[slot] = d; }
+                        if constexpr (LEAN) {
+                            best.valid = best.tri != kNoTriangle;
+                            best.opaque = 0u;
+                            if (best.valid) best.opaque = lds_word(lbvh.record(best.tri) + kLdsTriFlags) & 7u;
+                        }
                         a.b.hit[slot] = make_float4(best.t, best.u, best.v, __uint_as_float(best.valid ? (best.tri | ((best.opaque >> 1) << 29)) : 0xFFFFFFFFu));
                         if constexpr (TL) a.b.hitInst[slot] = best.inst;
                         active = false;
@@ -473,12 +500,14 @@
     static_assert(!TL || (!LDS_BVH && W == 4), "two-level structure: global 4-wide trees (every instance opaque: a shadow ray ends at its first hit)");
     static_assert(W != kQuantisedTree || (!LDS_BVH && !TL), "quantised nodes: flat tree in global memory");
     extern __shared__ __attribute__((aligned(128))) char smem[];
-    LdsStack<DEPTH, kExtendLdsStack> stack; LdsBvh<W> lbvh;
+    LdsStack<DEPTH, kExtendLdsStack> stack; LdsBvh<W, SHADOW> lbvh;
     constexpr size_t candBytes = SHADOW ? (size_t)kShadowCandidates * 2 * kBlock * 4 : 0;
     setup_lds<LDS_BVH, DEPTH, W>(smem, a.scene, stack, lbvh, candBytes);
     LdsCandidates cand; cand.base = reinterpret_cast<int32_t*>(smem + (size_t)LdsStack<DEPTH, kExtendLdsStack>::kRows * kBlock * 4) + threadIdx.x;
     if (DEPTH > kExtendLdsStack) { stack.spill = a.spill + blockIdx.x * kBlock + threadIdx.x; stack.spillStride = gridDim.x * kBlock; }
     typename GlobalBvhOf<(TL ? kTwoLevelTree : W)>::type gbvh = GlobalBvhOf<(TL ? kTwoLevelTree : W)>::make(a.scene);
+    typedef std::conditional_t<LDS_BVH, decltype(lbvh), typename GlobalBvhOf<(TL ? kTwoLevelTree : W)>::type> Bvh;
+    const Bvh& bvh = pick_bvh<LDS_BVH>(lbvh, gbvh);
     const SceneView& s = a.scene;
     const uint32_t wavesPerBlock = kBlock / 64;
     const uint32_t gw = uniform(blockIdx.x * wavesPerBlock + (threadIdx.x >> 6)), totalWaves = gridDim.x * wavesPerBlock;
@@ -494,7 +523,7 @@
     open_chunk();
     bool active = false;
     Ray r; r.o = mk3(0.0f, 0.0f, 0.0f); r.d = mk3(0.0f, 0.0f, 1.0f); r.tmin = 0.0f; r.tmax = 1e10f;
-    RayShear sh = make_shear(r.d); f3 inv = mk3(0.0f, 0.0f, 0.0f), noi = mk3(0.0f, 0.0f, 0.0f);
+    typename ShearOf<Bvh>::type sh = ray_shear(bvh, r); f3 inv = mk3(0.0f, 0.0f, 0.0f), noi = mk3(0.0f, 0.0f, 0.0f);
     HitKey lower; lower.have = false; lower.t = 0.0f; lower.inst = 0; lower.prim = 0;
     Hit best; best.valid = false; best.t = 0.0f; best.inst = 0; best.prim = 0; best.u = 0.0f; best.v = 0.0f; best.opaque = 0; best.tri = 0;
     int32_t cur = kTraversalDone; int sp = 0; uint64_t slot = 0; uint32_t rng = 0; float tlim = 0.0f;
@@ -514,7 +543,7 @@
                 if (SHADOW) r = shadow_ray(o, d, q1.w);
                 else { r.o = o; r.d = d; r.tmin = q0.w; r.tmax = q1.w; }
                 rng = rr; blocked = false; candOverflow = false; candCount = 0; lower.have = false; best.valid = false; tlim = r.tmax; sp = 0;
-                sh = make_shear(r.d);
+                sh = ray_shear(bvh, r);
                 if constexpr (TL) tl_world(tl, r); else { inv = traversal_rcp(r.d); noi = slab_origin_term(r.o, inv); }
                 cur = (emptyScene || !finite) ? kTraversalDone : (s.nodeCount == 0 ? s.rootLeaf : 0);
                 active = true;
@@ -550,29 +579,26 @@
                 }
             } else {
             while (cur >= 0) {
-                if (LDS_BVH) cur = inner_step(lbvh, cur, noi, inv, r.tmin, tlim, stack, sp);
-                else cur = inner_step(gbvh, cur, noi, inv, r.tmin, tlim, stack, sp);
+                cur = inner_step(bvh, cur, noi, inv, r.tmin, tlim, stack, sp);
                 if ((uint32_t)__popcll(__ballot(cur >= 0)) < a.nodeLoopMin) break;
             }
             if (cur < 0 && cur != kTraversalDone) {
                 const uint32_t enc = (uint32_t)(~cur), first = enc >> 2, count = (enc & 3u) + 1u;
                 for (uint32_t i = 0; i < count; ++i) {
-                    float4 ta, tb, tc;
-                    if (LDS_BVH) lbvh.tri(first + i, ta, tb, tc); else gbvh.tri(first + i, ta, tb, tc);
+                    typename TriWordsOf<Bvh>::type w;
                     float t, u, v;
-                    if (tri_test(mk3(ta.x, ta.y, ta.z), mk3(tb.x, tb.y, tb.z), mk3(tc.x, tc.y, tc.z), r, sh, t, u, v)) {
+                    if (leaf_test(bvh, first + i, r, sh, t, u, v, w)) {
                         if (SHADOW) {
-                            if (__float_as_uint(tc.w) & 1u) { blocked = true; break; }
-                            if (LDS_BVH) candidate_insert<kShadowCandidates>(lbvh, cand, candCount, candOverflow, t, first + i, __float_as_uint(ta.w), __float_as_uint(tb.w));
-                            else candidate_insert<kShadowCandidates>(gbvh, cand, candCount, candOverflow, t, first + i, __float_as_uint(ta.w), __float_as_uint(tb.w));
+                            if (w.flags() & 1u) { blocked = true; break; }
+                            candidate_insert<kShadowCandidates>(bvh, cand, candCount, candOverflow, t, first + i, w.inst(), w.prim());
                             continue;
                         }
-                        const uint32_t inst = __float_as_uint(ta.w), prim = __float_as_uint(tb.w);
+                        const uint32_t inst = w.inst(), prim = w.prim();
                         const bool ok = !lower.have || key_less(lower.t, lower.inst, lower.prim, t, inst, prim);
                         const bool take = ok && (!best.valid || key_less(t, inst, prim, best.t, best.inst, best.prim));
                         best.t = take ? t : best.t; best.u = take ? u : best.u; best.v = take ? v : best.v;
                         best.inst = take ? inst : best.inst; best.prim = take ? prim : best.prim; best.tri = take ? first + i : best.tri;
-                        best.opaque = take ? (__float_as_uint(tc.w) & 1u) : best.opaque;
+                        best.opaque = take ? (w.flags() & 1u) : best.opaque;
                         best.valid = best.valid || take;
                         tlim = take ? t : tlim;
                     }
@@ -589,8 +615,7 @@
                         if (blocked) vis = 0.0f;
                         else if (candCount > 0) {
                             if constexpr (TL) vis = shadow_retrace_two_level(s, gbvh, r, stack);
-                            else if (LDS_BVH) vis = shadow_resolve_candidates(s, lbvh, r, sh, candCount, candOverflow, cand, stack);
-                            else vis = shadow_resolve_candidates(s, gbvh, r, sh, candCount, candOverflow, cand, stack);
+                            else vis = shadow_resolve_candidates(s, bvh, r, sh, candCount, candOverflow, cand, stack);
                         }
                     }
                     out.t = vis; out.hit = vis < 1.0f ? 1u : 0u;
@@ -956,7 +981,7 @@
     constexpr bool SLIM = MODE == kShadowSlim;
     constexpr int kLdsMax = MODE == kShadowResolve ? kExtendLdsStack : kShadowLdsStack;
     extern __shared__ __attribute__((aligned(128))) char smem[];
-    LdsStack<DEPTH, kLdsMax> stack; LdsBvh<W> lbvh;
+    LdsStack<DEPTH, kLdsMax> stack; LdsBvh<W, (MODE != kShadowResolve)> lbvh;
     constexpr size_t candBytes = MODE == kShadowBuffered ? (size_t)kShadowCandidates * 2 * kBlock * 4 : 0;
     setup_lds<LDS_BVH, DEPTH, W>(smem, a.scene, stack, lbvh, candBytes);
     if (DEPTH > kLdsMax) { stack.spill = a.spill[1] + blockIdx.x * kBlock + threadIdx.x; stack.spillStride = gridDim.x * kBlock; }
@@ -1037,8 +1062,8 @@
                             Ray sr = shadow_ray(origin, L, maxDist);
                             GlobalCandidates gc; gc.base = a.b.sqCand + (size_t)(e * a.maxLights + j) * kShadowCandidates;
                             const int cnt = (int)((vis >> 8) & 0xFFu); const bool ovf = (vis >> 16) & 1u;
-                            if (LDS_BVH) shadow = shadow_resolve_candidates(s, lbvh, sr, make_shear(sr.d), cnt, ovf, gc, stack);
-                            else shadow = shadow_resolve_candidates(s, gbvh, sr, make_shear(sr.d), cnt, ovf, gc, stack);
+                            if (LDS_BVH) shadow = shadow_resolve_candidates(s, lbvh, sr, ray_shear(lbvh, sr), cnt, ovf, gc, stack);
+                            else shadow = shadow_resolve_candidates(s, gbvh, sr, ray_shear(gbvh, sr), cnt, ovf, gc, stack);
                         }
                     } else if (MODE == kShadowBuffered) {
                         if (LDS_BVH) shadow = shadow_query_buffered<kShadowCandidates>(s, lbvh, origin, L, maxDist, stack, cand);
diff --git a/hobbyrenderer_amd/csrc/tri_forms_check.cpp b/hobbyrenderer_amd/csrc/tri_forms_check.cpp
--- /dev/null
+++ b/hobbyrenderer_amd/csrc/tri_forms_check.cpp
@@ -0,0 +1,171 @@
+#include <cmath>
+#include <cstdint>
+#include <cstdio>
+#include <cstdlib>
+#include <cstring>
+#include <limits>
+#include <vector>
+
+#include "../../include/hobbyrt/tri_forms.h"
+
+namespace {
+struct Rng {
+    uint64_t s;
+    uint64_t next() { uint64_t z = (s += 0x9E3779B97F4A7C15ull); z = (z ^ (z >> 30)) * 0xBF58476D1CE4E5B9ull; z = (z ^ (z >> 27)) * 0x94D049BB133111EBull; return z ^ (z >> 31); }
+    float uni(float lo, float hi) { return lo + (hi - lo) * (float)((next() >> 40) * (1.0 / 16777216.0)); }
+};
+struct Tri { float p[3][3]; };
+struct Result { int hit; float t, u, v; };
+struct Tally { uint64_t cases = 0, hits = 0, mismatches = 0, unswappedDiffers = 0, unswappedBeyondZeroSign = 0; };
+
+uint32_t bits(float f) { uint32_t u; std::memcpy(&u, &f, 4); return u; }
+bool same(const Result& a, const Result& b) { return a.hit == b.hit && (!a.hit || (bits(a.t) == bits(b.t) && bits(a.u) == bits(b.u) && bits(a.v) == bits(b.v))); }
+
+void component_major(const Tri& t, float rec[12])
+{
+    for (int j = 0; j < 3; ++j) for (int c = 0; c < 3; ++c) rec[3 * c + j] = t.p[j][c];
+    rec[9] = rec[10] = rec[11] = 0.0f;
+}
+Result reference_form(const Tri& tr, const float* o, const float* d, float tmin, float tmax)
+{
+    int kz = 0;
+    if (std::fabs(d[1]) > std::fabs(d[kz])) kz = 1;
+    if (std::fabs(d[2]) > std::fabs(d[kz])) kz = 2;
+    int kx = (kz + 1) % 3, ky = (kx + 1) % 3;
+    if (d[kz] < 0.0f) { int t = kx; kx = ky; ky = t; }
+    const float Sx = d[kx] / d[kz], Sy = d[ky] / d[kz], Sz = 1.0f / d[kz];
+    float a[3], b[3], c[3];
+    for (int k = 0; k < 3; ++k) { a[k] = tr.p[0][k] - o[k]; b[k] = tr.p[1][k] - o[k]; c[k] = tr.p[2][k] - o[k]; }
+    const float Ax = a[kx] - Sx * a[kz], Ay = a[ky] - Sy * a[kz];
+    const float Bx = b[kx] - Sx * b[kz], By = b[ky] - Sy * b[kz];
+    const float Cx = c[kx] - Sx * c[kz], Cy = c[ky] - Sy * c[kz];
+    const float U = Cx * By - Cy * Bx, V = Ax * Cy - Ay * Cx, W = Bx * Ay - By * Ax;
+    Result r = { 0, 0.0f, 0.0f, 0.0f };
+    if ((U < 0.0f || V < 0.0f || W < 0.0f) && (U > 0.0f || V > 0.0f || W > 0.0f)) return r;
+    const float det = (U + V) + W;
+    if (det == 0.0f) return r;
+    const float Az = Sz * a[kz], Bz = Sz * b[kz], Cz = Sz * c[kz];
+    const float T = (U * Az + V * Bz) + W * Cz;
+    const float rcp = 1.0f / det, tt = T * rcp;
+    if (!(tt > tmin && tt < tmax)) return r;
+    r.hit = 1; r.t = tt; r.u = V * rcp; r.v = W * rcp;
+    return r;
+}
+Result picked_form(const Tri& t, const float* o, const float* d, float tmin, float tmax, bool exchange)
+{
+    HrtTriShear s = hrt_tri_shear(d[0], d[1], d[2]);
+    if (!exchange) s = hrt_tri_shear_axes(d[0], d[1], d[2], (s.kz + 1) % 3, (s.kz + 2) % 3, s.kz);
+    Result r = { 0, 0.0f, 0.0f, 0.0f };
+    r.hit = hrt_tri_test_picked(t.p[0], t.p[1], t.p[2], o, &s, tmin, tmax, &r.t, &r.u, &r.v);
+    return r;
+}
+Result rows_form(const Tri& t, const float* o, const float* d, float tmin, float tmax)
+{
+    float rec[12]; component_major(t, rec);
+    const HrtTriRows rows = hrt_tri_rows(o[0], o[1], o[2], d[0], d[1], d[2]);
+    const char* base = reinterpret_cast<const char*>(rec);
+    float x[3], y[3], z[3];
+    std::memcpy(x, base + rows.rx, 12); std::memcpy(y, base + rows.ry, 12); std::memcpy(z, base + rows.rz, 12);
+    Result r = { 0, 0.0f, 0.0f, 0.0f };
+    r.hit = hrt_tri_test_rows(x, y, z, &rows, tmin, tmax, &r.t, &r.u, &r.v);
+    return r;
+}
+int g_reported = 0;
+Result check(Tally& tally, const Tri& t, const float* o, const float* d, float tmin, float tmax)
+{
+    const Result a = reference_form(t, o, d, tmin, tmax), b = picked_form(t, o, d, tmin, tmax, true), c = rows_form(t, o, d, tmin, tmax);
+    const Result n = picked_form(t, o, d, tmin, tmax, false);
+    ++tally.cases; tally.hits += a.hit ? 1 : 0;
+    if (!same(a, n)) {
+        ++tally.unswappedDiffers;
+        const uint32_t sign = 0x80000000u;
+        const bool zeroSignOnly = a.hit && n.hit && a.t == n.t && a.u == n.u && a.v == n.v && ((bits(a.t) ^ bits(n.t)) | (bits(a.u) ^ bits(n.u)) | (bits(a.v) ^ bits(n.v))) == sign;
+        if (!zeroSignOnly) ++tally.unswappedBeyondZeroSign;
+    }
+    if (!same(a, b) || !same(a, c)) {
+        ++tally.mismatches;
+        if (g_reported++ < 10)
+            std::fprintf(stderr, "mismatch: o (%a %a %a) d (%a %a %a) [%a, %a] reference %d %a %a %a picked %d %a %a %a rows %d %a %a %a\n", o[0], o[1], o[2], d[0], d[1], d[2],
+                         tmin, tmax, a.hit, a.t, a.u, a.v, b.hit, b.t, b.u, b.v, c.hit, c.t, c.u, c.v);
+    }
+    return a;
+}
+
+void random_pairs(Tally& tally, uint64_t n, uint64_t seed)
+{
+    Rng g = { seed };
+    for (uint64_t i = 0; i < n; ++i) {
+        Tri t; float o[3], d[3];
+        for (int j = 0; j < 3; ++j) for (int c = 0; c < 3; ++c) t.p[j][c] = g.uni(-1.0f, 1.0f);
+        for (int c = 0; c < 3; ++c) o[c] = g.uni(-1.0f, 1.0f);
+        const float a = g.uni(-0.25f, 1.0f), b = g.uni(-0.25f, 1.0f), w = (1.0f - a) - b;
+        const uint64_t kind = g.next() % 10u;
+        const float scale = kind == 0 ? -g.uni(0.25f, 4.0f) : g.uni(0.25f, 4.0f);
+        for (int c = 0; c < 3; ++c) d[c] = (((a * t.p[0][c] + b * t.p[1][c]) + w * t.p[2][c]) - o[c]) * scale;
+        float tmin = 0.0f, tmax = 1e10f;
+        if (kind == 1) { const float at = 1.0f / scale; tmin = at * g.uni(0.5f, 1.05f); tmax = at * g.uni(0.95f, 2.0f); }
+        check(tally, t, o, d, tmin, tmax);
+    }
+}
+
+void constructed(Tally& tally)
+{
+    const float comps[] = { 1.0f, -1.0f, 0.5f, -0.5f, 0.25f, -0.25f, 0.0f, -0.0f };
+    const float e[][3] = { { 1, 0, 0 }, { 0, 1, 0 }, { 0, 0, 1 }, { 1, 1, 0 }, { 0, 1, 1 }, { 1, 0, 1 }, { 1, -1, 2 }, { -2, 1, 1 }, { 1, 1, 1 }, { 3, -2, -1 } };
+    const int ne = (int)(sizeof e / sizeof e[0]);
+    const float origins[][3] = { { 0, 0, 0 }, { 1, -2, 3 }, { -0.0f, 4, -0.0f }, { -3, -1, -2 } };
+    std::vector<Tri> tris;
+    for (const float* o : origins) for (float dx : comps) for (float dy : comps) for (float dz : comps) {
+        const float d[3] = { dx, dy, dz };
+        float q[3]; for (int c = 0; c < 3; ++c) q[c] = o[c] + d[c] * 4.0f;
+        tris.clear();
+        for (int i = 0; i < ne; ++i) for (int j = 0; j < ne; ++j) {
+            if (i == j) continue;
+            Tri t;
+            for (int c = 0; c < 3; ++c) { t.p[0][c] = q[c] - e[i][c] - e[j][c]; t.p[1][c] = q[c] + 2.0f * e[i][c] - e[j][c]; t.p[2][c] = q[c] - e[i][c] + 2.0f * e[j][c]; }
+            tris.push_back(t);
+            for (int v = 0; v < 3; ++v) {
+                for (int c = 0; c < 3; ++c) { t.p[v][c] = q[c]; t.p[(v + 1) % 3][c] = q[c] + e[i][c]; t.p[(v + 2) % 3][c] = q[c] + e[j][c]; }
+                tris.push_back(t);
+            }
+            for (int c = 0; c < 3; ++c) { t.p[0][c] = q[c] - e[i][c]; t.p[1][c] = q[c] + e[i][c]; t.p[2][c] = q[c] + e[j][c]; }
+            tris.push_back(t);
+            for (int c = 0; c < 3; ++c) { t.p[0][c] = q[c] + e[i][c]; t.p[1][c] = q[c] - e[i][c]; t.p[2][c] = q[c] - e[j][c]; }
+            tris.push_back(t);
+            for (int c = 0; c < 3; ++c) { t.p[0][c] = q[c] - e[i][c]; t.p[1][c] = q[c]; t.p[2][c] = q[c] + 2.0f * e[i][c]; }
+            tris.push_back(t);
+            for (int c = 0; c < 3; ++c) { t.p[0][c] = q[c] - d[c]; t.p[1][c] = q[c] + d[c]; t.p[2][c] = q[c] + e[i][c]; }
+            tris.push_back(t);
+        }
+        for (const Tri& t : tris) {
+            const Result r = check(tally, t, o, d, 0.0f, 1e10f);
+            if (r.hit) {
+                check(tally, t, o, d, r.t, 1e10f); check(tally, t, o, d, 0.0f, r.t);
+                check(tally, t, o, d, std::nextafter(r.t, 0.0f), std::nextafter(r.t, 1e10f));
+            }
+        }
+    }
+    const float nan = std::numeric_limits<float>::quiet_NaN(), inf = std::numeric_limits<float>::infinity();
+    const Tri t = { { { -1, -1, 2 }, { 3, -1, 2 }, { -1, 3, 2 } } };
+    for (int c = 0; c < 3; ++c) for (float bad : { nan, -nan, inf, -inf, 1e-42f, -1e-42f }) {
+        float o[3] = { 0, 0, 0 }, d[3] = { 0.25f, -0.25f, 1.0f };
+        d[c] = bad; check(tally, t, o, d, 0.0f, 1e10f);
+        d[c] = c == 2 ? 1.0f : 0.25f; o[c] = bad; check(tally, t, o, d, 0.0f, 1e10f);
+        const float dd[3] = { c == 0 ? bad : 0.0f, c == 1 ? bad : 0.0f, c == 2 ? bad : 0.0f }, oo[3] = { 0, 0, 0 };
+        check(tally, t, oo, dd, 0.0f, 1e10f);
+    }
+}
+}
+
+int main(int argc, char** argv)
+{
+    const uint64_t n = argc > 1 ? std::strtoull(argv[1], nullptr, 10) : 10000000ull, seed = argc > 2 ? std::strtoull(argv[2], nullptr, 10) : 20240607ull;
+    Tally rnd, con;
+    random_pairs(rnd, n, seed);
+    constructed(con);
+    std::printf("random pairs %llu hits %llu mismatches %llu unswapped_differs %llu constructed cases %llu hits %llu mismatches %llu unswapped_differs %llu beyond_zero_sign %llu\n",
+                (unsigned long long)rnd.cases, (unsigned long long)rnd.hits, (unsigned long long)rnd.mismatches, (unsigned long long)rnd.unswappedDiffers,
+                (unsigned long long)con.cases, (unsigned long long)con.hits, (unsigned long long)con.mismatches, (unsigned long long)con.unswappedDiffers,
+                (unsigned long long)(rnd.unswappedBeyondZeroSign + con.unswappedBeyondZeroSign));
+    return rnd.mismatches || con.mismatches ? 1 : 0;
+}
diff --git a/include/hobbyrt/tri_forms.h b/include/hobbyrt/tri_forms.h
--- /dev/null
+++ b/include/hobbyrt/tri_forms.h
@@ -0,0 +1,78 @@
+#ifndef HOBBYRT_TRI_FORMS_H
+#define HOBBYRT_TRI_FORMS_H
+
+#include "detmath.h"
+
+typedef struct { int kx, ky, kz; float Sx, Sy, Sz; } HrtTriShear;
+typedef struct { uint32_t rx, ry, rz; float ox, oy, oz; float Sx, Sy, Sz; } HrtTriRows;
+
+HRT_FN float hrt_tri_pick(float x, float y, float z, int k) { return k == 0 ? x : (k == 1 ? y : z); }
+
+HRT_FN HrtTriShear hrt_tri_shear_axes(float dx, float dy, float dz, int kx, int ky, int kz)
+{
+    HrtTriShear s;
+    s.kx = kx; s.ky = ky; s.kz = kz;
+    float m = hrt_tri_pick(dx, dy, dz, kz);
+    s.Sx = hrt_tri_pick(dx, dy, dz, kx) / m; s.Sy = hrt_tri_pick(dx, dy, dz, ky) / m; s.Sz = 1.0f / m;
+    return s;
+}
+HRT_FN HrtTriShear hrt_tri_shear(float dx, float dy, float dz)
+{
+    int kz = 0;
+    if (hrt_abs(dy) > hrt_abs(hrt_tri_pick(dx, dy, dz, kz))) kz = 1;
+    if (hrt_abs(dz) > hrt_abs(hrt_tri_pick(dx, dy, dz, kz))) kz = 2;
+    int kx = (kz + 1) % 3, ky = (kx + 1) % 3;
+    if (hrt_tri_pick(dx, dy, dz, kz) < 0.0f) { int t = kx; kx = ky; ky = t; }
+    return hrt_tri_shear_axes(dx, dy, dz, kx, ky, kz);
+}
+
+HRT_FN int hrt_tri_core(float Akx, float Aky, float Akz, float Bkx, float Bky, float Bkz, float Ckx, float Cky, float Ckz,
+                        float Sx, float Sy, float Sz, float tmin, float tmax, float* t, float* u, float* v)
+{
+    float Ax = Akx - Sx * Akz, Ay = Aky - Sy * Akz;
+    float Bx = Bkx - Sx * Bkz, By = Bky - Sy * Bkz;
+    float Cx = Ckx - Sx * Ckz, Cy = Cky - Sy * Ckz;
+    float U = Cx * By - Cy * Bx;
+    float V = Ax * Cy - Ay * Cx;
+    float W = Bx * Ay - By * Ax;
+    if ((U < 0.0f || V < 0.0f || W < 0.0f) && (U > 0.0f || V > 0.0f || W > 0.0f)) return 0;
+    float det = (U + V) + W;
+    if (det == 0.0f) return 0;
+    float Az = Sz * Akz, Bz = Sz * Bkz, Cz = Sz * Ckz;
+    float T = (U * Az + V * Bz) + W * Cz;
+    float rcp = 1.0f / det;
+    float tt = T * rcp;
+    if (!(tt > tmin && tt < tmax)) return 0;
+    *t = tt; *u = V * rcp; *v = W * rcp;
+    return 1;
+}
+
+HRT_FN int hrt_tri_test_picked(const float* p0, const float* p1, const float* p2, const float* o, const HrtTriShear* s,
+                               float tmin, float tmax, float* t, float* u, float* v)
+{
+    const float Ax = p0[0] - o[0], Ay = p0[1] - o[1], Az = p0[2] - o[2];
+    const float Bx = p1[0] - o[0], By = p1[1] - o[1], Bz = p1[2] - o[2];
+    const float Cx = p2[0] - o[0], Cy = p2[1] - o[1], Cz = p2[2] - o[2];
+    return hrt_tri_core(hrt_tri_pick(Ax, Ay, Az, s->kx), hrt_tri_pick(Ax, Ay, Az, s->ky), hrt_tri_pick(Ax, Ay, Az, s->kz),
+                        hrt_tri_pick(Bx, By, Bz, s->kx), hrt_tri_pick(Bx, By, Bz, s->ky), hrt_tri_pick(Bx, By, Bz, s->kz),
+                        hrt_tri_pick(Cx, Cy, Cz, s->kx), hrt_tri_pick(Cx, Cy, Cz, s->ky), hrt_tri_pick(Cx, Cy, Cz, s->kz),
+                        s->Sx, s->Sy, s->Sz, tmin, tmax, t, u, v);
+}
+
+HRT_FN HrtTriRows hrt_tri_rows(float ox, float oy, float oz, float dx, float dy, float dz)
+{
+    const HrtTriShear s = hrt_tri_shear(dx, dy, dz);
+    HrtTriRows r;
+    r.rx = 12u * (uint32_t)s.kx; r.ry = 12u * (uint32_t)s.ky; r.rz = 12u * (uint32_t)s.kz;
+    r.ox = hrt_tri_pick(ox, oy, oz, s.kx); r.oy = hrt_tri_pick(ox, oy, oz, s.ky); r.oz = hrt_tri_pick(ox, oy, oz, s.kz);
+    r.Sx = s.Sx; r.Sy = s.Sy; r.Sz = s.Sz;
+    return r;
+}
+HRT_FN int hrt_tri_test_rows(const float* x, const float* y, const float* z, const HrtTriRows* r,
+                             float tmin, float tmax, float* t, float* u, float* v)
+{
+    return hrt_tri_core(x[0] - r->ox, y[0] - r->oy, z[0] - r->oz, x[1] - r->ox, y[1] - r->oy, z[1] - r->oz,
+                        x[2] - r->ox, y[2] - r->oy, z[2] - r->oz, r->Sx, r->Sy, r->Sz, tmin, tmax, t, u, v);
+}
+
+#endif
```
